# zsc/MOSS-TTSD

Measured on AMD Instinct MI355X. Metric: audio codec tokens/sec/node (decode, bf16, batch 32 @ 4k ctx), higher is better.
Workload: dtype bf16; 1 GPU; configs[2]: batch 32 synthetic dialogues/GPU, 4k-token KV context, top-k/top-p sampling on 8 channels, decode steps at full context; batch_per_gpu=32, context=4096, prompt=512, layers=28, hidden=2048, parallelism=dp1 (batch shard, no per-step collective)

## Files before the change

include/mtts.h:

```cpp
#ifndef MTTS_H
#define MTTS_H

#include <stdint.h>

#ifdef __cplusplus
extern "C" {
#endif

#define MTTS_OK 0
#define MTTS_EINVAL (-1)
#define MTTS_EHIP (-2)
#define MTTS_ENOMEM (-3)
#define MTTS_ESTATE (-4)

#define MTTS_CHANNELS 8

typedef struct MttsConfig {
    int32_t vocab_size;
    int32_t hidden_size;
    int32_t intermediate_size;
    int32_t num_hidden_layers;
    int32_t num_attention_heads;
    int32_t num_key_value_heads;
    int32_t head_dim;
// ... 66 lines not shown
                      const MttsSamplerCfg* sampler, uint64_t seed,
                      int64_t* host_out_ids, int32_t out_capacity, int32_t* out_len,
                      const int64_t* host_forced, int32_t forced_len, int64_t* host_decisions,
                      void* stream);

int32_t mtts_begin(MttsEngine* e, const int64_t* host_input_ids, const uint8_t* host_attention_mask,
                   int32_t B, int32_t T, int32_t max_length,
                   const MttsSamplerCfg* sampler, uint64_t seed, void* stream);
int32_t mtts_step(MttsEngine* e, int32_t n_steps, void* stream);
int32_t mtts_sync_state(MttsEngine* e, int32_t* steps_done, int32_t* all_finished, void* stream);
int32_t mtts_read_generated(MttsEngine* e, int64_t* host_gen, int32_t capacity_steps, int32_t* n_steps);
int32_t mtts_set_output_scores(MttsEngine* e, int32_t on);
int32_t mtts_read_scores(MttsEngine* e, float* host_lp, int32_t capacity_steps, int32_t* n_steps);
int32_t mtts_slot_read_scores(MttsEngine* e, int32_t slot, float* host_rows, int32_t capacity_steps, int32_t* n_steps);
int32_t mtts_set_top_logprobs(MttsEngine* e, int32_t k);
int32_t mtts_read_top_logprobs(MttsEngine* e, float* host_logp, int32_t* host_top_ids, float* host_top_logp,
                               int32_t capacity_steps, int32_t* n_steps);
int32_t mtts_slot_read_top_logprobs(MttsEngine* e, int32_t slot, float* host_logp, int32_t* host_top_ids, float* host_top_logp,
                                    int32_t capacity_steps, int32_t* n_steps);
int32_t mtts_score(MttsEngine* e, const int64_t* host_input_ids, const uint8_t* host_attention_mask,
                   const int64_t* host_labels, int32_t B, int32_t T, float* host_logp, void* stream);
#define MTTS_SCORE_MAX_TOPK 16
#define MTTS_SCORE_TOPK_ROWS 512
int32_t mtts_score_topk(MttsEngine* e, const int64_t* host_input_ids, const uint8_t* host_attention_mask,
                        const int64_t* host_labels, int32_t B, int32_t T, float* host_logp, int32_t k,
                        int32_t* host_top_ids, float* host_top_logp, void* stream);
int32_t mtts_read_logits(MttsEngine* e, uint16_t* host_logits0, uint16_t* host_logits17, void* stream);
int32_t mtts_read_logits_f32(MttsEngine* e, float* host_logits0, float* host_logits17, void* stream);
int32_t mtts_sched_open(MttsEngine* e, int32_t B, int32_t gen_cap, const MttsSamplerCfg* sampler, void* stream);
int32_t mtts_slot_submit(MttsEngine* e, int32_t slot, const int64_t* host_ids, int32_t T, int32_t max_length, uint64_t seed,
                         void* stream);
int32_t mtts_slot_submit_row(MttsEngine* e, int32_t slot, const int64_t* host_ids, int32_t T, int32_t max_length, uint64_t seed,
                             int32_t row_id, void* stream);
int32_t mtts_set_row_ids(MttsEngine* e, const int32_t* host_row_ids, int32_t n);
int32_t mtts_set_takes(MttsEngine* e, int32_t n);
int32_t mtts_set_sampler_floors(MttsEngine* e, const MttsSamplerFloors floors[8] );
int32_t mtts_set_sampler_bans(MttsEngine* e, const MttsSamplerBans bans[8] );
int32_t mtts_set_sampler_typical(MttsEngine* e, const float typical_p[8] );
int64_t mtts_debug_ban_launches(void);
int32_t mtts_slot_fork(MttsEngine* e, int32_t src_slot, int32_t dst_slot, uint64_t seed, int32_t row_id, void* stream);
int32_t mtts_slot_states(MttsEngine* e, int32_t* host_state, void* stream);
int32_t mtts_slot_read(MttsEngine* e, int32_t slot, int64_t* host_rows, int32_t capacity_steps, int32_t* n_steps);
int32_t mtts_read_seq_state(MttsEngine* e, int32_t* host_nas, int32_t* host_unfinished, int32_t* host_kv_len, void* stream);
int32_t mtts_slot_evict(MttsEngine* e, int32_t slot, void* stream);
int32_t mtts_kv_pool_state(MttsEngine* e, int32_t* total_pages, int32_t* free_pages, int32_t* max_pages_per_seq);
int32_t mtts_read_page_table(MttsEngine* e, int32_t* host_table, int32_t* host_n_pages);
int32_t mtts_set_forced_mode(MttsEngine* e, int32_t as_draw);
int32_t mtts_debug_read_device_page_table(MttsEngine* e, int32_t* host_table, void* stream);
int32_t mtts_export_codes(MttsEngine* e, int32_t first, int32_t n, int64_t* dev_codes, void* stream);
int32_t mtts_profile_enable(MttsEngine* e, int32_t on);
int32_t mtts_profile_read(MttsEngine* e, int32_t which, double* total_ms, int64_t* launches, int64_t* bytes);

int32_t mtts_debug_set_kv_len(MttsEngine* e, int32_t kv_len);
int32_t mtts_debug_kv_pack_stats(MttsEngine* e, int64_t* out6);
int32_t mtts_debug_step_plan(MttsEngine* e, int32_t pages_bound, char* buf, int32_t cap);
int32_t mtts_k_attn_bench(MttsEngine* e, int32_t phase, int32_t iters, float* avg_ms, int64_t* bytes_per_launch);
int32_t mtts_k_gemm_bench(int32_t N, int32_t K, int32_t epi, int32_t ksplit, int32_t waves, int32_t copies,
                          int32_t iters, float* avg_us);

int32_t mtts_debug_wseal_stats(MttsEngine* e, int64_t* out12);
int64_t mtts_debug_wseal_launches(void);
int32_t mtts_k_gemm_sealed_bench(const void* dev_w, int32_t N, int32_t K, int32_t epi, int32_t ksplit, int32_t copies,
                                 int32_t iters, int32_t sealed, int32_t head_form, float* avg_us, int64_t* out2);

int32_t mtts_k_wseal(const void* dev_packed, int32_t ntiles, int32_t K, int32_t ktw, void* dev_sealed, void* stream);
int32_t mtts_k_gemm_sealed(const void* dev_w, const void* dev_x, void* dev_out, int32_t M, int32_t N, int32_t K, int32_t epi,
                           int32_t ksplit, int32_t sealed, int32_t head_form, int64_t* out2, void* stream);
int32_t mtts_k_gemm_bf16(const void* dev_w, const void* dev_x, void* dev_y,
                         int32_t M, int32_t N, int32_t K, int32_t ksplit, void* stream);
int64_t mtts_debug_gemm_depth_launches(void);
int64_t mtts_debug_fold_norm_launches(void);
int32_t mtts_k_oproj_resid(const void* dev_wo, const void* dev_attn, void* dev_x, void* dev_x_packed, int32_t R, int32_t N,
                           void* stream);
int32_t mtts_k_fold_pair(const void* dev_wo, const void* dev_attn, void* dev_x, const void* dev_norm_w, const void* dev_wgu,
                         float eps, int32_t R, int32_t N_gu, void* dev_y, void* stream);
int32_t mtts_k_bf16_round_check(int64_t* out2, void* stream);
int32_t mtts_k_fold_bench(int32_t N_gu, int32_t copies, int32_t iters, int32_t mode, float* avg_us);
int64_t mtts_debug_attn_row_launches(void);
int32_t mtts_k_attn_section(const float* dev_slabs, int32_t ksplit, const void* dev_qnw, const void* dev_knw, const void* dev_cos,
                            const void* dev_sin, float eps, const void* dev_k, const void* dev_v, const int32_t* host_lens,
                            const int32_t* host_page_table, int32_t R, int32_t Lmax, int32_t nq, int32_t nkv, int32_t sealed,
                            int32_t path, void* dev_out, void* dev_kcache, void* dev_vcache, void* dev_kpack, void* dev_vpack,
                            void* stream);
int32_t mtts_k_attn_prefill(const float* dev_slabs, int32_t ksplit, const void* dev_qnw, const void* dev_knw, const void* dev_cos,
                            const void* dev_sin, float eps, const void* dev_k, const void* dev_v, const int32_t* host_lens,
                            const int32_t* host_cached, const int32_t* host_page_table, int32_t B, int32_t Lmax, int32_t nq,
                            int32_t nkv, void* dev_out, void* dev_q, void* dev_kcache, void* dev_vcache, void* stream);
int32_t mtts_k_gemm_swiglu_bf16(const void* dev_w, const void* dev_x, void* dev_y,
                                int32_t M, int32_t N, int32_t K, void* stream);
int32_t mtts_k_rmsnorm(const void* dev_x, const void* dev_w, void* dev_y,
                       int32_t rows, int32_t n, float eps, void* stream);
int32_t mtts_k_embed_norm(const int32_t* host_tokens, const int32_t* host_seq, const void* const* host_tables,
                          const int32_t* host_vocab, const void* dev_norm_w, int32_t R, int32_t H, float eps,
                          void* dev_x, void* dev_xn, void* stream);
int32_t mtts_k_resid_norm(const float* dev_slabs, int32_t ksplit, int32_t Npad, void* dev_x, const void* dev_norm_w,
                          const int32_t* host_seq, const int32_t* host_last, int32_t R, int32_t H, int32_t nseq, float eps,
                          void* dev_xn, void* dev_hlast, void* stream);
int32_t mtts_k_gemv_small(int32_t epi, int32_t pro, const void* dev_w, int32_t rows, int32_t N, int32_t K, int32_t want_ksplit,
                          const void* dev_x_in, const float* dev_slabs, int32_t slab_ksplit, const void* dev_norm_w, float eps,
                          void* dev_x_out, const float* dev_opart, const int32_t* host_seq, const int32_t* host_pos, int32_t nq,
                          int32_t nchunks_max, const void* dev_xrows, void* dev_y, int32_t* out_plan, void* stream);
int32_t mtts_k_gemm_tile(int32_t epi, const void* dev_w, const void* dev_x, void* dev_y, int32_t M, int32_t N, int32_t K,
                         int32_t ksplit, void* stream);
int32_t mtts_k_rope_kvwrite(const void* dev_qkv, const int32_t* host_pos, const void* dev_qnorm, const void* dev_knorm,
                            const void* dev_cos, const void* dev_sin, int32_t R, int32_t nq, int32_t nkv, float eps,
                            void* dev_q, void* dev_k, void* dev_v, void* stream);
int32_t mtts_k_paged_attn_decode(const void* dev_q, const void* dev_k, const void* dev_v, const int32_t* host_lens,
                                 const int32_t* host_page_table, int32_t R, int32_t Lmax, int32_t nq, int32_t nkv,
                                 void* dev_out, void* stream);
int32_t mtts_k_kv_seal(const void* dev_pages, int32_t npages, void* dev_sealed, int32_t as_k, void* stream);
int32_t mtts_k_head_ce(const void* dev_w, const void* dev_x, const int32_t* host_labels, int32_t M, int32_t N, int32_t K,
                       int32_t n_valid, int32_t segments, float* dev_logp, void* stream);
int32_t mtts_k_head_topk(const void* dev_w, const void* dev_x, int32_t M, int32_t N, int32_t K, int32_t n_valid,
                         int32_t segments, int32_t k, int32_t* dev_ids, float* dev_logp, void* stream);
int32_t mtts_k_lora_pack(const void* dev_base, int32_t rows, int32_t cols, const float* dev_lora_a, const float* dev_lora_b,
                         int32_t r, float scaling, int32_t rows_pad, int32_t row_mul, int32_t row_off, int32_t dtype,
                         void* dev_out, void* stream);
int32_t mtts_k_lora_delta(const void* dev_x, int32_t R, int32_t K, int32_t Npad, int32_t nseg, const int32_t* host_segs,
                          int32_t n_adapters, const void* const* host_a, const void* const* host_b, const int32_t* host_r,
                          const float* host_scaling, const int32_t* host_row_adapter, float* dev_slabs, int32_t ks, void* stream);
int32_t mtts_k_swiglu_slabs(const void* dev_w, const void* dev_x, const float* dev_delta, void* dev_y, float* dev_slab0_out,
                            int32_t M, int32_t N, int32_t K, void* stream);
int32_t mtts_k_sample(const void* dev_logits_bf16, int32_t rows, int32_t vocab,
                      const void* dev_history_bitmap, const MttsSamplerCfg* cfg,
                      int32_t mask_id, uint64_t seed, int32_t step, int32_t channel,
                      int32_t* dev_tokens, void* stream);
int32_t mtts_k_sample_scores(const void* dev_logits_bf16, int32_t rows, int32_t vocab,
                             const void* dev_history_bitmap, const MttsSamplerCfg* cfg,
                             int32_t mask_id, uint64_t seed, int32_t step, int32_t channel,
                             int32_t* dev_tokens, float* dev_logp, void* stream);
int32_t mtts_k_sample_floors(const void* dev_logits_bf16, int32_t rows, int32_t vocab,
                             const void* dev_history_bitmap, const MttsSamplerCfg* cfg,
                             int32_t mask_id, uint64_t seed, int32_t step, int32_t channel,
                             int32_t* dev_tokens, float* dev_logp, const MttsSamplerFloors* floors, void* stream);
int32_t mtts_k_sample_bans(const void* dev_logits_bf16, int32_t rows, int32_t vocab,
                           const void* dev_history_bitmap, const MttsSamplerCfg* cfg,
                           int32_t mask_id, uint64_t seed, int32_t step, int32_t channel,
                           int32_t* dev_tokens, float* dev_logp, const MttsSamplerFloors* floors, const void* dev_ban,
                           void* stream);
int32_t mtts_k_sample_typical(const void* dev_logits_bf16, int32_t rows, int32_t vocab,
                              const void* dev_history_bitmap, const MttsSamplerCfg* cfg,
                              int32_t mask_id, uint64_t seed, int32_t step, int32_t channel,
                              int32_t* dev_tokens, float* dev_logp, const MttsSamplerFloors* floors, const void* dev_ban,
                              float typical_p, void* stream);
int32_t mtts_k_ngram_ban(const int32_t* dev_hist, const int32_t* dev_lens, int32_t rows, int32_t cap, int32_t n,
                         const int32_t* host_static, int32_t n_static, int32_t vocab, int32_t eos_id, int32_t eos_on,
                         void* dev_ban, void* stream);
int32_t mtts_k_gen_topk(const void* dev_logits, int32_t is_f32, int32_t rows, int32_t vocab, int32_t mask_id,
                        const int32_t* dev_decisions, int32_t k, float* dev_logp, int32_t* dev_top_ids, float* dev_top_logp,
                        void* stream);

typedef struct MttsCodecConfig {
    int32_t nq, codebook_size, rvq_dim, quant_out_dim;
    int32_t adapter_layers, adapter_dim, adapter_heads, adapter_ffn, adapter_max_pos;
    int32_t up_stride;
    int32_t dec_layers, dec_dim, dec_heads, dec_ffn, dec_max_pos, mel_bins;
    int32_t voc_dim, voc_inter, voc_layers, n_fft, hop;
    int32_t mel_n_fft, mel_hop, mel_frames;
    int32_t enc_layers, enc_dim, enc_heads, enc_ffn, enc_max_pos;
    int32_t sem_adapter_layers, pre_rvq_layers, down_pool;
} MttsCodecConfig;

typedef struct MttsCodec MttsCodec;
const char* mtts_codec_last_error(void);
int32_t mtts_codec_create(const MttsCodecConfig* cfg, int32_t device, MttsCodec** out);
int32_t mtts_codec_destroy(MttsCodec* c);
// ... 42 lines not shown
```

moss-ttsd_amd/csrc/attn.hip:

```cpp
#include "launch.h"
#include <algorithm>
#include <atomic>
#include <cstdlib>
#ifndef MTTS_PK_WAVES
#define MTTS_PK_WAVES 0
#endif
#if MTTS_PK_WAVES
#define PK_OCC(PK) __attribute__((amdgpu_waves_per_eu((PK) ? MTTS_PK_WAVES : 1, (PK) ? MTTS_PK_WAVES : 8)))
#else
#define PK_OCC(PK)
#endif

#include "seal.h"

__device__ bool seal_lane_k(const u32x4_t* __restrict__ raw, u32x4_t* __restrict__ pk, uint8_t* __restrict__ lds, int lane) {
    u32x4_t v[16];
#pragma unroll
    for (int j = 0; j < 16; ++j) v[j] = raw[j * 64];
    __builtin_amdgcn_wave_barrier();
    uint32_t* row = (uint32_t*)(lds + lane * 128);
#pragma unroll
    for (int j = 0; j < 16; ++j)
#pragma unroll
        for (int c = 0; c < 4; c += 2) {
            const uint32_t a = u4c(v[j], c), b = u4c(v[j], c + 1);
            row[2 * j + (c >> 1)] = ((a >> 7) & 0xffu) | (((a >> 23) & 0xffu) << 8) | (((b >> 7) & 0xffu) << 16) | (((b >> 23) & 0xffu) << 24);
        }
    __builtin_amdgcn_wave_barrier();
    uint32_t a0 = 0u, a1 = 0u, n0 = 0u, n1 = 0u;
    for (int t = 0; t < 64; ++t) {
        const uint32_t e = *(const uint16_t*)(lds + t * 128 + 2 * lane);
        a0 += e & 0xffu; n0 += (e & 0xffu) ? 1u : 0u;
        a1 += e >> 8; n1 += (e >> 8) ? 1u : 0u;
    }
    const int s0 = n0 ? min(max((int)((a0 + n0 / 2) / n0) - 125, -127), 127) : 0;
    const int s1 = n1 ? min(max((int)((a1 + n1 / 2) / n1) - 125, -127), 127) : 0;
    int8_t* sv = (int8_t*)(lds + 8192);
    sv[2 * lane] = (int8_t)s0;
    sv[2 * lane + 1] = (int8_t)s1;
    __builtin_amdgcn_wave_barrier();
    bool unfit = false;
#pragma unroll
    for (int j = 0; j < 16; ++j) {
        uint32_t w[4] = {v[j].x, v[j].y, v[j].z, v[j].w};
#pragma unroll
        for (int c = 0; c < 4; ++c) {
            const uint32_t sh = *(const uint16_t*)(sv + 8 * j + 2 * c);
            uint32_t out = 0u;
#pragma unroll
            for (int h = 0; h < 2; ++h) {
                uint32_t b = (w[c] >> (16 * h)) & 0xffffu;
                const int sft = (int)(int8_t)((sh >> (8 * h)) & 0xffu);
                const int e = (int)((b >> 7) & 0xffu);
                if (e == 0) {
                    if ((b & 0x7fu) && sft) unfit = true;
                } else {
                    const int e2 = e - sft;
                    if (e == 255 ? sft != 0 : (e2 < 1 || e2 > 254)) unfit = true;
                    else b = (b - ((uint32_t)sft << 7)) & 0xffffu;
                }
                out |= b << (16 * h);
            }
            w[c] = out;
        }
        v[j] = u32x4_t{w[0], w[1], w[2], w[3]};
    }
    return seal_encode(v, pk, ((uint32_t)s0 & 0xffu) | (((uint32_t)s1 & 0xffu) << 8), unfit);
}
__device__ bool seal_lane_v(const u32x4_t* __restrict__ raw, u32x4_t* __restrict__ pk, uint8_t* __restrict__ lds, int lane) {
    u32x4_t v[16];
#pragma unroll
    for (int j = 0; j < 16; ++j) v[j] = raw[j * 64];
    const int sub = lane >> 5;
    __builtin_amdgcn_wave_barrier();
    uint32_t* row = (uint32_t*)(lds + lane * 128);
#pragma unroll
    for (int it = 0; it < 16; ++it)
#pragma unroll
        for (int h = 0; h < 2; ++h) {
            uint32_t sum = 0u, cnt = 0u;
#pragma unroll
            for (int c = 0; c < 4; ++c) {
                const uint32_t e = (u4c(v[it], c) >> (7 + 16 * h)) & 0xffu;
                sum += e;
                cnt += e ? 1u : 0u;
            }
            row[2 * it + h] = sum | (cnt << 16);
        }
    __builtin_amdgcn_wave_barrier();
    int mean;
    {
        const int t = lane, st = (t >> 1) & 1, j = 2 * (t >> 2) + (t & 1);
        uint32_t tot = 0u, cn = 0u;
        for (int d = 0; d < 32; ++d) {
            const uint32_t w = ((const uint32_t*)(lds + (st * 32 + d) * 128))[j];
            tot += w & 0xffffu;
// ... 66 lines not shown
                              : seal_lane_k(kcache + layer * raw_layer + pi * (MTTS_PAGE * MTTS_HD / 8) + lane,
                                            kpack + layer * pk_layer + pi * (MTTS_PKU * 64) + lane, klds, lane);
        seal_count(fit, cnt, layer, wave, lane);
    }
}
__global__ __launch_bounds__(128) void kv_seal_all_kernel(const u32x4_t* __restrict__ kcache, const u32x4_t* __restrict__ vcache,
                                                          u32x4_t* __restrict__ kpack, u32x4_t* __restrict__ vpack, int total_pages,
                                                          size_t raw_layer, size_t pk_layer, unsigned long long* __restrict__ cnt) {
    __shared__ __attribute__((aligned(16))) uint8_t klds[8192 + 128];
    __shared__ __attribute__((aligned(16))) uint8_t vlds[8192 + 320];
    const int kvh = blockIdx.y, layer = blockIdx.z, wave = threadIdx.x >> 6, lane = threadIdx.x & 63;
    const size_t pi = (size_t)kvh * total_pages + blockIdx.x;
    const bool fit = wave ? seal_lane_v(vcache + layer * raw_layer + pi * (MTTS_PAGE * MTTS_HD / 8) + lane,
                                        vpack + layer * pk_layer + pi * (MTTS_PKU * 64) + lane, vlds, lane)
                          : seal_lane_k(kcache + layer * raw_layer + pi * (MTTS_PAGE * MTTS_HD / 8) + lane,
                                        kpack + layer * pk_layer + pi * (MTTS_PKU * 64) + lane, klds, lane);
    seal_count(fit, cnt, layer, wave, lane);
}
__global__ __launch_bounds__(64) void kv_seal_pages_kernel(const u32x4_t* __restrict__ raw, u32x4_t* __restrict__ pk, int as_k) {
    __shared__ __attribute__((aligned(16))) uint8_t klds[8192 + 320];
    const u32x4_t* src = raw + (size_t)blockIdx.x * (MTTS_PAGE * MTTS_HD / 8) + threadIdx.x;
    u32x4_t* dst = pk + (size_t)blockIdx.x * (MTTS_PKU * 64) + threadIdx.x;
    if (as_k == 1) seal_lane_k(src, dst, klds, threadIdx.x);
    else if (as_k == 2) seal_lane_v(src, dst, klds, threadIdx.x);
    else seal_lane(src, dst);
}
void launch_kv_seal_pages(const void* raw, void* pk, int npages, int as_k, hipStream_t st) {
    hipLaunchKernelGGL(kv_seal_pages_kernel, dim3(npages), dim3(64), 0, st, (const u32x4_t*)raw, (u32x4_t*)pk, as_k);
}
__global__ __launch_bounds__(64) void kv_pack_count_kernel(const u32x4_t* __restrict__ kpack, const u32x4_t* __restrict__ vpack,
                                                           const int32_t* __restrict__ page_table, const int32_t* __restrict__ complete,
                                                           int max_pages, int total_pages, size_t pk_layer, unsigned long long* __restrict__ out) {
    const int b = blockIdx.x, kvh = blockIdx.y, layer = blockIdx.z, lane = threadIdx.x;
    unsigned long long n = 0, dk = 0, dv = 0;
    for (int pg = 0; pg < complete[b]; ++pg) {
        const size_t pi = (size_t)kvh * total_pages + page_table[(size_t)b * max_pages + pg];
        const u32x4_t fk = kpack[layer * pk_layer + pi * (MTTS_PKU * 64) + 12 * 64 + lane];
        const u32x4_t fv = vpack[layer * pk_layer + pi * (MTTS_PKU * 64) + 12 * 64 + lane];
        n += 1;
        dk += __any(fk.w != 0u) ? 1 : 0;
        dv += __any(fv.w != 0u) ? 1 : 0;
    }
    if (lane == 0 && n) {
        atomicAdd(out + 0, n); atomicAdd(out + 1, dk); atomicAdd(out + 2, n); atomicAdd(out + 3, dv);
    }
}
void launch_kv_pack_count(const void* kpack, const void* vpack, const int32_t* page_table, const int32_t* complete, int B, int max_pages,
                          int total_pages, int nkv, int L, unsigned long long* out, hipStream_t st) {
    const size_t pk_layer = (size_t)total_pages * nkv * (MTTS_PKU * 64);
    hipLaunchKernelGGL(kv_pack_count_kernel, dim3(B, nkv, L), dim3(64), 0, st, (const u32x4_t*)kpack, (const u32x4_t*)vpack, page_table,
                       complete, max_pages, total_pages, pk_layer, out);
}
void launch_kv_seal_rows(const void* kcache, const void* vcache, void* kpack, void* vpack, const int32_t* page_table,
                         const RowMeta* meta, int R, int max_pages, int total_pages, int nkv, int L, unsigned long long* cnt, hipStream_t st) {
    const size_t raw_layer = (size_t)total_pages * nkv * (MTTS_PAGE * MTTS_HD / 8), pk_layer = (size_t)total_pages * nkv * (MTTS_PKU * 64);
    hipLaunchKernelGGL(kv_seal_scan_kernel, dim3((R + 63) / 64, nkv, L), dim3(128), 0, st, (const u32x4_t*)kcache, (const u32x4_t*)vcache,
                       (u32x4_t*)kpack, (u32x4_t*)vpack, page_table, meta, R, max_pages, total_pages, raw_layer, pk_layer, cnt);
}
void launch_kv_seal_all(const void* kcache, const void* vcache, void* kpack, void* vpack, int total_pages, int nkv, int L,
                        unsigned long long* cnt, hipStream_t st) {
    const size_t raw_layer = (size_t)total_pages * nkv * (MTTS_PAGE * MTTS_HD / 8), pk_layer = (size_t)total_pages * nkv * (MTTS_PKU * 64);
    hipLaunchKernelGGL(kv_seal_all_kernel, dim3(total_pages, nkv, L), dim3(128), 0, st, (const u32x4_t*)kcache, (const u32x4_t*)vcache,
                       (u32x4_t*)kpack, (u32x4_t*)vpack, total_pages, raw_layer, pk_layer, cnt);
}


__device__ __forceinline__ void fuse_reduce(const QkvFuse& f, int r, int col, int lane, float& a, float& b) {
    const size_t kstride = (size_t)MTTS_PFCAP * f.Npad;
    const float* p0 = f.partial + (size_t)r * f.Npad + col + lane;
    a = 0.f; b = 0.f;
    for (int k0 = 0; k0 < f.ksplit; k0 += 8) {
        float ta[8], tb[8];
#pragma unroll
        for (int j = 0; j < 8; ++j) {
            const float* pk = p0 + (size_t)min(k0 + j, f.ksplit - 1) * kstride;
            ta[j] = pk[0];
            tb[j] = pk[64];
        }
        if (k0 == 0) { a = ta[0]; b = tb[0]; }
#pragma unroll
        for (int j = 0; j < 8; ++j)
            if (k0 + j < f.ksplit && k0 + j > 0) { a += ta[j]; b += tb[j]; }
    }
    a = rbf(a);
    b = rbf(b);
}

__device__ __forceinline__ void fuse_reduce_request(const QkvFuse& f, int r, int col, int lane, float (&ta)[8], float (&tb)[8]) {
    const size_t kstride = (size_t)MTTS_PFCAP * f.Npad;
    const float* p0 = f.partial + (size_t)r * f.Npad + col + lane;
#pragma unroll
    for (int j = 0; j < 8; ++j) {
        const float* pk = p0 + (size_t)min(j, f.ksplit - 1) * kstride;
        ta[j] = pk[0];
        tb[j] = pk[64];
    }
}
__device__ __forceinline__ void fuse_reduce_sum(const QkvFuse& f, const float (&ta)[8], const float (&tb)[8], float& a, float& b) {
    a = ta[0]; b = tb[0];
#pragma unroll
    for (int j = 1; j < 8; ++j)
        if (j < f.ksplit) { a += ta[j]; b += tb[j]; }
    a = rbf(a);
    b = rbf(b);
}

struct FuseVec { float w0, w1, c, s; };
__device__ __forceinline__ FuseVec fuse_load_vec(const QkvFuse& f, const uint16_t* __restrict__ nw, int pos, int lane) {
    FuseVec v;
    v.w0 = bf2f(nw[lane]);
    v.w1 = bf2f(nw[lane + 64]);
    v.c = bf2f(f.rope_cos[(size_t)pos * 64 + lane]);
    v.s = bf2f(f.rope_sin[(size_t)pos * 64 + lane]);
    return v;
}
__device__ __forceinline__ void fuse_norm_rope(const QkvFuse& f, const FuseVec& v, float a, float b, float& o1, float& o2) {
    const float ss = wave_sum(a * a + b * b);
    const float inv = 1.0f / sqrtf(ss / (float)MTTS_HD + f.eps);
    a = rbf(v.w0 * rbf(a * inv));
    b = rbf(v.w1 * rbf(b * inv));
    o1 = rbf(rbf(a * v.c) + rbf(-b * v.s));
    o2 = rbf(rbf(b * v.c) + rbf(a * v.s));
}

template <int G, bool FUSED, bool PK>
__global__ __launch_bounds__(256) PK_OCC(PK) void attn_scores_kernel(
    const uint16_t* __restrict__ qbuf, u32x4_t* __restrict__ kcache, const int32_t* __restrict__ page_table,
    const RowMeta* __restrict__ meta, uint16_t* __restrict__ scores, float* __restrict__ stats, int max_pages,
    int total_pages, int nq, int nkv, float scale, QkvFuse f, const u32x4_t* __restrict__ kpack) {
    __shared__ __attribute__((aligned(16))) uint32_t qs[G][MTTS_HD / 2];
    __shared__ __attribute__((aligned(16))) uint16_t knew[MTTS_HD];
    __shared__ __attribute__((aligned(16))) uint32_t qw[PK ? 4 : 1][G][MTTS_HD / 2];
    const int r = blockIdx.z, kvh = blockIdx.y;
    const RowMeta m = meta[r];
    if (m.seq < 0) return;
    const int len = m.pos + 1;
    const int npages = (len + MTTS_PAGE - 1) / MTTS_PAGE;
    if ((int)blockIdx.x * 4 >= npages) return;
    const int wave = __builtin_amdgcn_readfirstlane(threadIdx.x >> 6), lane = threadIdx.x & 63;
    const int pg = blockIdx.x * 4 + wave;
    const int own_pg = m.pos >> 6;
    const int Lmax = max_pages * MTTS_PAGE;
    uint32_t qreg[(G * MTTS_HD / 2 + 255) / 256];
    if (!FUSED) {
#pragma unroll
        for (int i = 0; i < (G * MTTS_HD / 2 + 255) / 256; ++i) {
            const int idx = threadIdx.x + 256 * i;
            qreg[i] = idx < G * MTTS_HD / 2 ? ((const uint32_t*)qbuf)[((size_t)r * nq + kvh * G) * (MTTS_HD / 2) + idx] : 0u;
        }
    }
    const bool own = FUSED && (own_pg >> 2) == (int)blockIdx.x;
    const bool pre = FUSED && f.ksplit <= 8 && wave < G + (own ? 1 : 0);
    float pta[8], ptb[8];
    FuseVec pfv{0.f, 0.f, 0.f, 0.f};
    if (pre) {
        const bool isk = wave == G;
        pfv = fuse_load_vec(f, isk ? f.knorm_w : f.qnorm_w, m.pos, lane);
        fuse_reduce_request(f, r, (isk ? nq + kvh : kvh * G + wave) * MTTS_HD, lane, pta, ptb);
    }
    const int page = pg < npages ? page_table[(size_t)m.seq * max_pages + pg] : 0;
    const u32x4_t* kp = kcache + ((size_t)kvh * total_pages + page) * (MTTS_PAGE * MTTS_HD / 8) + lane;

    auto stage_q = [&]() {
        if (FUSED) {
            for (int hh = wave; hh < G + (own ? 1 : 0); hh += 4) {
                const bool isk = hh == G;
                float a, b, o1, o2;
                FuseVec fv;
                if (pre && hh == wave) {
                    fv = pfv;
                    fuse_reduce_sum(f, pta, ptb, a, b);
                } else {
                    fv = fuse_load_vec(f, isk ? f.knorm_w : f.qnorm_w, m.pos, lane);
                    fuse_reduce(f, r, (isk ? nq + kvh : kvh * G + hh) * MTTS_HD, lane, a, b);
                }
                fuse_norm_rope(f, fv, a, b, o1, o2);
                if (!isk) {
                    ((uint16_t*)qs[hh])[lane] = f2bf(o1);
                    ((uint16_t*)qs[hh])[lane + 64] = f2bf(o2);
                } else {
                    knew[lane] = f2bf(o1);
                    knew[lane + 64] = f2bf(o2);
                    const int opage = page_table[(size_t)m.seq * max_pages + own_pg];
                    uint16_t* base = (uint16_t*)kcache + ((size_t)kvh * total_pages + opage) * (MTTS_PAGE * MTTS_HD);
                    const int tok = m.pos & 63;
                    base[(((lane >> 3) * 64) + tok) * 8 + (lane & 7)] = f2bf(o1);
                    base[((((lane + 64) >> 3) * 64) + tok) * 8 + (lane & 7)] = f2bf(o2);
                }
            }
        } else {
#pragma unroll
            for (int i = 0; i < (G * MTTS_HD / 2 + 255) / 256; ++i) {
                const int idx = threadIdx.x + 256 * i;
                if (idx < G * MTTS_HD / 2) (&qs[0][0])[idx] = qreg[i];
            }
        }
        __syncthreads();
    };
    auto finish = [&](const float* acc) {
        const int tok = pg * MTTS_PAGE + lane;
        const bool valid = tok < len;
#pragma unroll
        for (int g = 0; g < G; ++g) {
            const int h = kvh * G + g;
            float sc = rbf(rbf(acc[g]) * scale);
            if (valid) scores[((size_t)r * nq + h) * Lmax + tok] = f2bf(sc);
            float mx = wave_max(valid ? sc : -INFINITY);
            float e = valid ? expf(sc - mx) : 0.f;
            float sm = wave_sum(e);
            if (lane == 0) {
                float* st = stats + (((size_t)r * nq + h) * max_pages + pg) * 2;
                st[0] = mx;
                st[1] = sm;
            }
        }
    };
    auto raw_dots = [&](u32x4_t (&kv)[16]) {
        if (FUSED && pg == own_pg && lane == (m.pos & 63)) {
#pragma unroll
            for (int j = 0; j < 16; ++j) kv[j] = *(const u32x4_t*)&knew[8 * j];
        }
        float acc[G];
#pragma unroll
        for (int g = 0; g < G; ++g) acc[g] = 0.f;
#pragma unroll
        for (int j = 0; j < 16; ++j) {
#pragma unroll
            for (int g = 0; g < G; ++g) {
                const u32x4_t q = *(const u32x4_t*)&qs[g][4 * j];
                acc[g] = dot2bf(kv[j].x, q.x, acc[g]);
                acc[g] = dot2bf(kv[j].y, q.y, acc[g]);
                acc[g] = dot2bf(kv[j].z, q.z, acc[g]);
                acc[g] = dot2bf(kv[j].w, q.w, acc[g]);
            }
#pragma unroll
            for (int g = 0; g < G; ++g) asm volatile("" : "+v"(acc[g]));
            if ((j & 3) == 3) __builtin_amdgcn_sched_barrier(0);
        }
        finish(acc);
    };

    if (PK && pg < own_pg) {
        u32x4_t pk[MTTS_PKU];
        const u32x4_t* pp = kpack + ((size_t)kvh * total_pages + page) * (MTTS_PKU * 64) + lane;
#pragma unroll
        for (int j = 0; j < MTTS_PKU; ++j) pk[pk_order(j)] = __builtin_nontemporal_load(pp + pk_order(j) * 64);
        stage_q();
        bool qok = true;
        const uint32_t sh = pk[12].z;
#pragma unroll
        for (int g = 0; g < G; ++g) {
            const uint32_t qd = qs[g][lane];
            uint32_t out = 0u;
#pragma unroll
            for (int h = 0; h < 2; ++h) {
                uint32_t b = (qd >> (16 * h)) & 0xffffu;
                const int sft = (int)(int8_t)((sh >> (8 * h)) & 0xffu);
                if ((b & 0x7fffu) && sft) {
                    const int e = (int)((b >> 7) & 0xffu), e2 = e + sft;
                    if (e == 0 || e == 255 || e2 < 1 || e2 > 254) qok = false;
                    else b = (b + ((uint32_t)sft << 7)) & 0xffffu;
                }
                out |= b << (16 * h);
            }
            qw[PK ? wave : 0][g][lane] = out;
        }
        __builtin_amdgcn_wave_barrier();
        if (__any(pk[12].w != 0u || !qok)) {
            u32x4_t kv[16];
#pragma unroll
            for (int j = 0; j < 16; ++j) kv[j] = __builtin_nontemporal_load(kp + j * 64);
            raw_dots(kv);
            return;
        }
        float acc[G];
#pragma unroll
        for (int g = 0; g < G; ++g) acc[g] = 0.f;
#pragma unroll
        for (int j = 0; j < 16; ++j) {
            uint32_t w[4];
            pk_unit(pk, j, w);
#pragma unroll
            for (int g = 0; g < G; ++g) {
                const u32x4_t q = *(const u32x4_t*)&qw[PK ? wave : 0][g][4 * j];
                acc[g] = dot2bf(w[0], q.x, acc[g]);
                acc[g] = dot2bf(w[1], q.y, acc[g]);
                acc[g] = dot2bf(w[2], q.z, acc[g]);
                acc[g] = dot2bf(w[3], q.w, acc[g]);
            }
#pragma unroll
            for (int g = 0; g < G; ++g) asm volatile("" : "+v"(acc[g]));
            if ((j & 3) == 3) __builtin_amdgcn_sched_barrier(0);
        }
        finish(acc);
    } else {
        u32x4_t kv[16];
#pragma unroll
        for (int j = 0; j < 16; ++j) kv[j] = __builtin_nontemporal_load(kp + j * 64);
        stage_q();
        if (pg >= npages) return;
        raw_dots(kv);
    }
}

template <int G, bool FUSED, bool PK, bool SF>
__global__ __launch_bounds__(PV_WAVES * 64) PK_OCC(PK) void attn_pv_kernel(
    const uint16_t* __restrict__ scores, const float* __restrict__ stats, u32x4_t* __restrict__ vcache,
    const int32_t* __restrict__ page_table, const RowMeta* __restrict__ meta, float* __restrict__ opart,
    int max_pages, int total_pages, int nchunks_max, int nq, int nkv, QkvFuse f, const u32x4_t* __restrict__ vpack) {
    __shared__ float red[PV_WAVES][G][MTTS_HD];
    __shared__ uint16_t pbuf[PV_WAVES][G][MTTS_PAGE];
    __shared__ __attribute__((aligned(16))) uint16_t vnew[MTTS_HD];
    const int r = blockIdx.z, kvh = blockIdx.y, chunk = blockIdx.x;
    const RowMeta m = meta[r];
    if (m.seq < 0) return;
    const int len = m.pos + 1;
    const int npages = (len + MTTS_PAGE - 1) / MTTS_PAGE;
    if (chunk * ATT_PB >= npages) return;
    const int wave = threadIdx.x >> 6, lane = threadIdx.x & 63;
    const int Lmax = max_pages * MTTS_PAGE;
    const int sub = lane >> 5, dl = lane & 31;
    float2 s0[G];
    if (SF) {
#pragma unroll
        for (int g = 0; g < G; ++g) {
            const float* st = stats + ((size_t)r * nq + kvh * G + g) * max_pages * 2;
            s0[g] = lane < npages ? *(const float2*)(st + 2 * lane) : float2{-INFINITY, 0.f};
        }
        __builtin_amdgcn_sched_barrier(0);
    }
    u32x4_t vv[16];
    int pg = chunk * ATT_PB + wave * (ATT_PB / PV_WAVES);
    const int own_pg = m.pos >> 6;
    bool packed = false;
    const u32x4_t* vp = nullptr;
    uint16_t sraw[G];
    auto load_page = [&]() {
        if (SF) {
            const int tok = pg * MTTS_PAGE + lane;
#pragma unroll
            for (int g = 0; g < G; ++g) sraw[g] = tok < len ? scores[((size_t)r * nq + kvh * G + g) * Lmax + tok] : (uint16_t)0;
            __builtin_amdgcn_sched_barrier(0);
        }
        const int page = page_table[(size_t)m.seq * max_pages + pg];
        vp = vcache + ((size_t)kvh * total_pages + page) * (MTTS_PAGE * MTTS_HD / 8) + lane;
        packed = PK && pg < own_pg;
        if (packed) {
            const u32x4_t* pp = vpack + ((size_t)kvh * total_pages + page) * (MTTS_PKU * 64) + lane;
#pragma unroll
            for (int it = 0; it < MTTS_PKU; ++it) vv[pk_order(it)] = __builtin_nontemporal_load(pp + pk_order(it) * 64);
        } else {
#pragma unroll
            for (int it = 0; it < 16; ++it) vv[it] = __builtin_nontemporal_load(vp + it * 64);
        }
    };
    const bool own_wave = FUSED && own_pg >= pg && own_pg < pg + ATT_PB / PV_WAVES;
    const bool pre_v = SF && own_wave && f.ksplit <= 8;
    float vta[8], vtb[8];
    if (pre_v) fuse_reduce_request(f, r, (nq + nkv + kvh) * MTTS_HD, lane, vta, vtb);
    if (pg < npages) load_page();
    if (own_wave) {
        float a, b;
        if (pre_v) fuse_reduce_sum(f, vta, vtb, a, b);
        else fuse_reduce(f, r, (nq + nkv + kvh) * MTTS_HD, lane, a, b);
        vnew[lane] = f2bf(a);
        vnew[lane + 64] = f2bf(b);
        const int page = page_table[(size_t)m.seq * max_pages + own_pg];
        const int tok = m.pos & 63;
        uint16_t* dst = (uint16_t*)vcache + ((size_t)kvh * total_pages + page) * (MTTS_PAGE * MTTS_HD) + (size_t)(tok >> 1) * (MTTS_HD * 2) + (tok & 1);
        dst[2 * lane] = f2bf(a);
        dst[2 * (lane + 64)] = f2bf(b);
    }
    float M[G], S[G];
#pragma unroll
    for (int g = 0; g < G; ++g) {
        const float* st = stats + ((size_t)r * nq + kvh * G + g) * max_pages * 2;
        float mx = -INFINITY;
        if (SF) mx = fmaxf(mx, s0[g].x);
        for (int p = lane + (SF ? 64 : 0); p < npages; p += 64) mx = fmaxf(mx, st[2 * p]);
        mx = wave_max(mx);
        float sm = 0.f;
        if (SF && lane < npages) sm += s0[g].y * expf(s0[g].x - mx);
        for (int p = lane + (SF ? 64 : 0); p < npages; p += 64) sm += st[2 * p + 1] * expf(st[2 * p] - mx);
        sm = wave_sum(sm);
        M[g] = mx;
        S[g] = sm;
    }
    float acc[G][4];
#pragma unroll
    for (int g = 0; g < G; ++g)
#pragma unroll
        for (int i = 0; i < 4; ++i) acc[g][i] = 0.f;
#pragma unroll 1
    for (int pp = 0; pp < ATT_PB / PV_WAVES; ++pp, ++pg) {
        if (pg >= npages) break;
        if (pp > 0) load_page();
        if (own_wave && pg == own_pg) {
            __builtin_amdgcn_wave_barrier();
            const int tp = (m.pos & 63) >> 1;
            if (sub == (tp & 1)) {
                const uint32_t w01 = ((const uint32_t*)vnew)[2 * dl], w23 = ((const uint32_t*)vnew)[2 * dl + 1];
                const uint32_t nv[4] = {w01 & 0xffffu, w01 >> 16, w23 & 0xffffu, w23 >> 16};
                const bool hi = m.pos & 1;
#pragma unroll
                for (int it = 0; it < 16; ++it)
                    if (it == (tp >> 1)) {
                        vv[it].x = hi ? (vv[it].x & 0xffffu) | (nv[0] << 16) : (vv[it].x & 0xffff0000u) | nv[0];
                        vv[it].y = hi ? (vv[it].y & 0xffffu) | (nv[1] << 16) : (vv[it].y & 0xffff0000u) | nv[1];
                        vv[it].z = hi ? (vv[it].z & 0xffffu) | (nv[2] << 16) : (vv[it].z & 0xffff0000u) | nv[2];
                        vv[it].w = hi ? (vv[it].w & 0xffffu) | (nv[3] << 16) : (vv[it].w & 0xffff0000u) | nv[3];
                    }
            }
        }
        uint16_t pun[G];
        bool pok = true;
        {
            const int tok = pg * MTTS_PAGE + lane;
            const int sv = (PK && packed) ? (int)(vv[12].z & 0xffu) : 0;
#pragma unroll
            for (int g = 0; g < G; ++g) {
                float p = 0.f;
                if (tok < len) {
                    float s = bf2f(SF ? sraw[g] : scores[((size_t)r * nq + kvh * G + g) * Lmax + tok]);
                    p = expf(s - M[g]) / S[g];
                }
                uint32_t pb = f2bf(p);
                pun[g] = (uint16_t)pb;
                if (sv && (pb & 0x7fffu)) {
                    if (((pb >> 7) & 0xffu) == 0u) pok = false;
                    else pb += (uint32_t)sv << 7;
                }
                pbuf[wave][g][lane] = (uint16_t)pb;
            }
        }
        __builtin_amdgcn_wave_barrier();
        if (PK && packed && __any(vv[12].w != 0u || !pok)) {
            packed = false;
#pragma unroll
            for (int it = 0; it < 16; ++it) vv[it] = __builtin_nontemporal_load(vp + it * 64);
#pragma unroll
            for (int g = 0; g < G; ++g) pbuf[wave][g][lane] = pun[g];
            __builtin_amdgcn_wave_barrier();
        }
        if (PK && packed) {
#pragma unroll
            for (int it = 0; it < 16; ++it) {
                uint32_t w[4];
                pk_unit(vv, it, w);
#pragma unroll
                for (int g = 0; g < G; ++g) {
                    const uint32_t pp2 = ((const uint32_t*)&pbuf[wave][g][0])[it * 2 + sub];
                    acc[g][0] = dot2bf(w[0], pp2, acc[g][0]);
                    acc[g][1] = dot2bf(w[1], pp2, acc[g][1]);
                    acc[g][2] = dot2bf(w[2], pp2, acc[g][2]);
                    acc[g][3] = dot2bf(w[3], pp2, acc[g][3]);
                }
            }
        } else {
#pragma unroll
            for (int it = 0; it < 16; ++it) {
#pragma unroll
                for (int g = 0; g < G; ++g) {
                    const uint32_t pp2 = ((const uint32_t*)&pbuf[wave][g][0])[it * 2 + sub];
                    acc[g][0] = dot2bf(vv[it].x, pp2, acc[g][0]);
                    acc[g][1] = dot2bf(vv[it].y, pp2, acc[g][1]);
                    acc[g][2] = dot2bf(vv[it].z, pp2, acc[g][2]);
                    acc[g][3] = dot2bf(vv[it].w, pp2, acc[g][3]);
                }
            }
        }
        __builtin_amdgcn_wave_barrier();
    }
#pragma unroll
    for (int g = 0; g < G; ++g)
#pragma unroll
        for (int i = 0; i < 4; ++i) {
            float v = acc[g][i];
            v = add_xor32(v);
            if (sub == 0) red[wave][g][dl * 4 + i] = v;
        }
    __syncthreads();
    for (int i = threadIdx.x; i < G * MTTS_HD; i += PV_WAVES * 64) {
        int g = i / MTTS_HD, d = i % MTTS_HD;
        float v = red[0][g][d];
#pragma unroll
        for (int w = 1; w < PV_WAVES; ++w) v += red[w][g][d];
        opart[(((size_t)r * nq + kvh * G + g) * nchunks_max + chunk) * MTTS_HD + d] = v;
    }
}

__global__ __launch_bounds__(512) void attn_combine_kernel(const float* __restrict__ opart, const RowMeta* __restrict__ meta,
                                                           uint16_t* __restrict__ out_packed, int nchunks_max, int nq,
                                                           int pages_per_chunk) {
    const int r = blockIdx.x, h = blockIdx.y * 4 + (threadIdx.x >> 7), d = threadIdx.x & 127;
    if (h >= nq) return;
    const RowMeta m = meta[r];
    float s = 0.f;
    const int npages = m.seq >= 0 ? (m.pos + 1 + MTTS_PAGE - 1) / MTTS_PAGE : 0;
    const int nch = (npages + pages_per_chunk - 1) / pages_per_chunk;
    const float* p = opart + ((size_t)r * nq + h) * nchunks_max * MTTS_HD + d;
    for (int c0 = 0; c0 < nch; c0 += 8) {
        float t[8];
#pragma unroll
        for (int j = 0; j < 8; ++j) t[j] = p[(size_t)min(c0 + j, nch - 1) * MTTS_HD];
#pragma unroll
        for (int j = 0; j < 8; ++j)
            if (c0 + j < nch) s += t[j];
    }
    out_packed[xpack_off(r, h * MTTS_HD + d, nq * MTTS_HD)] = f2bf(s);
}

static_assert(ROW_WAVES >= 6 && ROW_WAVES <= 16, "one wave per q head + the K row + the V row; at most 1024 threads");
static std::atomic<long long> g_row_launches{0};
long long mtts_attn_row_launches() { return g_row_launches.load(); }

template <int G, bool PK>
__global__ __launch_bounds__(ROW_WAVES * 64) void attn_row_kernel(
    u32x4_t* __restrict__ kcache, u32x4_t* __restrict__ vcache, const int32_t* __restrict__ page_table,
    const RowMeta* __restrict__ meta, uint16_t* __restrict__ out_packed, int npb, int max_pages, int total_pages, int nq,
    int nkv, float scale, QkvFuse f, const u32x4_t* __restrict__ kpack, const u32x4_t* __restrict__ vpack) {
    constexpr int W = ROW_WAVES;
    extern __shared__ __attribute__((aligned(16))) uint8_t row_lds[];
    uint32_t* qs = (uint32_t*)row_lds;
    uint16_t* knew = (uint16_t*)(row_lds + G * 256);
    uint16_t* vnew = knew + MTTS_HD;
    uint32_t* qw = (uint32_t*)(row_lds + G * 256 + 512);
    uint16_t* pbuf = (uint16_t*)((uint8_t*)qw + (PK ? W * G * 256 : 0));
    float2* st = (float2*)((uint8_t*)pbuf + W * G * 128);
    uint16_t* sc = (uint16_t*)(st + G * npb);
    float* items = (float*)(sc + (size_t)G * npb * MTTS_PAGE);
    const int r = blockIdx.y, kvh = blockIdx.x;
    const RowMeta m = meta[r];
    if (m.seq < 0) {
        for (int i = threadIdx.x; i < G * MTTS_HD; i += W * 64) out_packed[xpack_off(r, kvh * G * MTTS_HD + i, nq * MTTS_HD)] = f2bf(0.f);
        return;
    }
    const int len = m.pos + 1;
    const int npages = min((len + MTTS_PAGE - 1) / MTTS_PAGE, npb);
    const int nch = (npages + ATT_PB - 1) / ATT_PB;
    const int wave = __builtin_amdgcn_readfirstlane(threadIdx.x >> 6), lane = threadIdx.x & 63;
    const int own_pg = m.pos >> 6;
    const int sub = lane >> 5, dl = lane & 31;
    const int32_t* ptab = page_table + (size_t)m.seq * max_pages;

    const bool epi = wave < G + 2;
    const int vw = epi ? wave + W - (G + 2) : wave - (G + 2);
    if (epi) {
        const int col = (wave < G ? kvh * G + wave : wave == G ? nq + kvh : nq + nkv + kvh) * MTTS_HD;
        FuseVec pfv{0.f, 0.f, 0.f, 0.f};
        if (wave <= G) pfv = fuse_load_vec(f, wave == G ? f.knorm_w : f.qnorm_w, m.pos, lane);
        float a, b;
        if (f.ksplit <= 8) {
            float pta[8], ptb[8];
            fuse_reduce_request(f, r, col, lane, pta, ptb);
            fuse_reduce_sum(f, pta, ptb, a, b);
        } else fuse_reduce(f, r, col, lane, a, b);
        const int opage = ptab[own_pg], tok = m.pos & 63;
        if (wave <= G) {
            float o1, o2;
            fuse_norm_rope(f, pfv, a, b, o1, o2);
            if (wave < G) {
                ((uint16_t*)(qs + wave * 64))[lane] = f2bf(o1);
                ((uint16_t*)(qs + wave * 64))[lane + 64] = f2bf(o2);
            } else {
                knew[lane] = f2bf(o1);
                knew[lane + 64] = f2bf(o2);
                uint16_t* base = (uint16_t*)kcache + ((size_t)kvh * total_pages + opage) * (MTTS_PAGE * MTTS_HD);
                base[(((lane >> 3) * 64) + tok) * 8 + (lane & 7)] = f2bf(o1);
                base[((((lane + 64) >> 3) * 64) + tok) * 8 + (lane & 7)] = f2bf(o2);
            }
        } else {
            vnew[lane] = f2bf(a);
            vnew[lane + 64] = f2bf(b);
            uint16_t* dst = (uint16_t*)vcache + ((size_t)kvh * total_pages + opage) * (MTTS_PAGE * MTTS_HD) + (size_t)(tok >> 1) * (MTTS_HD * 2) + (tok & 1);
            dst[2 * lane] = f2bf(a);
            dst[2 * (lane + 64)] = f2bf(b);
        }
        __builtin_amdgcn_sched_barrier(0);
    }
    auto stage = [&]() { __syncthreads(); };

    auto finish = [&](int pg, const float* acc) {
        const int tok = pg * MTTS_PAGE + lane;
        const bool valid = tok < len;
#pragma unroll
        for (int g = 0; g < G; ++g) {
            float s = rbf(rbf(acc[g]) * scale);
            if (valid) sc[(size_t)g * npb * MTTS_PAGE + tok] = f2bf(s);
            float mx = wave_max(valid ? s : -INFINITY);
            float e = valid ? expf(s - mx) : 0.f;
            float sm = wave_sum(e);
            if (lane == 0) st[g * npb + pg] = float2{mx, sm};
        }
    };
    auto raw_dots = [&](int pg, u32x4_t (&kv)[16]) {
        if (pg == own_pg && lane == (m.pos & 63)) {
#pragma unroll
            for (int j = 0; j < 16; ++j) kv[j] = *(const u32x4_t*)&knew[8 * j];
        }
        float acc[G];
#pragma unroll
        for (int g = 0; g < G; ++g) acc[g] = 0.f;
#pragma unroll
        for (int j = 0; j < 16; ++j) {
#pragma unroll
            for (int g = 0; g < G; ++g) {
                const u32x4_t q = *(const u32x4_t*)&qs[g * 64 + 4 * j];
                acc[g] = dot2bf(kv[j].x, q.x, acc[g]);
                acc[g] = dot2bf(kv[j].y, q.y, acc[g]);
                acc[g] = dot2bf(kv[j].z, q.z, acc[g]);
                acc[g] = dot2bf(kv[j].w, q.w, acc[g]);
            }
#pragma unroll
            for (int g = 0; g < G; ++g) asm volatile("" : "+v"(acc[g]));
            if ((j & 3) == 3) __builtin_amdgcn_sched_barrier(0);
        }
        finish(pg, acc);
    };
    auto k_page = [&](int pg, bool first) {
        const int page = ptab[pg];
        const u32x4_t* kp = kcache + ((size_t)kvh * total_pages + page) * (MTTS_PAGE * MTTS_HD / 8) + lane;
        if (PK && pg < own_pg) {
            u32x4_t pk[MTTS_PKU];
            const u32x4_t* pp = kpack + ((size_t)kvh * total_pages + page) * (MTTS_PKU * 64) + lane;
#pragma unroll
            for (int j = 0; j < MTTS_PKU; ++j) pk[pk_order(j)] = __builtin_nontemporal_load(pp + pk_order(j) * 64);
            if (first) stage();
            bool qok = true;
            const uint32_t sh = pk[12].z;
            uint32_t* qwv = qw + wave * G * 64;
            __builtin_amdgcn_wave_barrier();
#pragma unroll
            for (int g = 0; g < G; ++g) {
                const uint32_t qd = qs[g * 64 + lane];
                uint32_t out = 0u;
#pragma unroll
                for (int h = 0; h < 2; ++h) {
                    uint32_t b = (qd >> (16 * h)) & 0xffffu;
                    const int sft = (int)(int8_t)((sh >> (8 * h)) & 0xffu);
                    if ((b & 0x7fffu) && sft) {
                        const int e = (int)((b >> 7) & 0xffu), e2 = e + sft;
                        if (e == 0 || e == 255 || e2 < 1 || e2 > 254) qok = false;
                        else b = (b + ((uint32_t)sft << 7)) & 0xffffu;
                    }
                    out |= b << (16 * h);
                }
                qwv[g * 64 + lane] = out;
            }
            __builtin_amdgcn_wave_barrier();
            if (__any(pk[12].w != 0u || !qok)) {
                u32x4_t kv[16];
#pragma unroll
                for (int j = 0; j < 16; ++j) kv[j] = __builtin_nontemporal_load(kp + j * 64);
                raw_dots(pg, kv);
                return;
            }
            float acc[G];
#pragma unroll
            for (int g = 0; g < G; ++g) acc[g] = 0.f;
#pragma unroll
            for (int j = 0; j < 16; ++j) {
                uint32_t w[4];
                pk_unit(pk, j, w);
#pragma unroll
                for (int g = 0; g < G; ++g) {
                    const u32x4_t q = *(const u32x4_t*)&qwv[g * 64 + 4 * j];
                    acc[g] = dot2bf(w[0], q.x, acc[g]);
                    acc[g] = dot2bf(w[1], q.y, acc[g]);
                    acc[g] = dot2bf(w[2], q.z, acc[g]);
                    acc[g] = dot2bf(w[3], q.w, acc[g]);
                }
#pragma unroll
                for (int g = 0; g < G; ++g) asm volatile("" : "+v"(acc[g]));
                if ((j & 3) == 3) __builtin_amdgcn_sched_barrier(0);
            }
            finish(pg, acc);
        } else {
            u32x4_t kv[16];
#pragma unroll
            for (int j = 0; j < 16; ++j) kv[j] = __builtin_nontemporal_load(kp + j * 64);
            if (first) stage();
            raw_dots(pg, kv);
        }
    };
    if (vw < npages) k_page(vw, true);
    else stage();
#pragma unroll 1
    for (int pg = vw + W; pg < npages; pg += W) k_page(pg, false);

    u32x4_t vv[16];
    bool packed = false;
    const u32x4_t* vp = nullptr;
    auto load_page = [&](int pg) {
        const int page = ptab[pg];
        vp = vcache + ((size_t)kvh * total_pages + page) * (MTTS_PAGE * MTTS_HD / 8) + lane;
        packed = PK && pg < own_pg;
        if (packed) {
            const u32x4_t* pp = vpack + ((size_t)kvh * total_pages + page) * (MTTS_PKU * 64) + lane;
#pragma unroll
            for (int it = 0; it < MTTS_PKU; ++it) vv[pk_order(it)] = __builtin_nontemporal_load(pp + pk_order(it) * 64);
        } else {
#pragma unroll
            for (int it = 0; it < 16; ++it) vv[it] = __builtin_nontemporal_load(vp + it * 64);
        }
    };
    if (2 * wave < npages) load_page(2 * wave);
    __syncthreads();
    float M[G], S[G];
#pragma unroll
    for (int g = 0; g < G; ++g) {
        const float2* sg = st + g * npb;
        const float2 s0 = lane < npages ? sg[lane] : float2{-INFINITY, 0.f};
        float mx = -INFINITY;
        mx = fmaxf(mx, s0.x);
        for (int p = lane + 64; p < npages; p += 64) mx = fmaxf(mx, sg[p].x);
        mx = wave_max(mx);
        float sm = 0.f;
        if (lane < npages) sm += s0.y * expf(s0.x - mx);
        for (int p = lane + 64; p < npages; p += 64) sm += sg[p].y * expf(sg[p].x - mx);
        sm = wave_sum(sm);
        M[g] = mx;
        S[g] = sm;
    }
    uint16_t* pb = pbuf + wave * G * MTTS_PAGE;
#pragma unroll 1
    for (int item = wave; item < PV_WAVES * nch; item += W) {
        float acc[G][4];
#pragma unroll
        for (int g = 0; g < G; ++g)
#pragma unroll
            for (int i = 0; i < 4; ++i) acc[g][i] = 0.f;
#pragma unroll 1
        for (int pp = 0; pp < ATT_PB / PV_WAVES; ++pp) {
            const int pg = item * (ATT_PB / PV_WAVES) + pp;
            if (pg >= npages) break;
            if (pp > 0 || item != wave) load_page(pg);
            if (pg == own_pg) {
                const int tp = (m.pos & 63) >> 1;
                if (sub == (tp & 1)) {
                    const uint32_t w01 = ((const uint32_t*)vnew)[2 * dl], w23 = ((const uint32_t*)vnew)[2 * dl + 1];
                    const uint32_t nv[4] = {w01 & 0xffffu, w01 >> 16, w23 & 0xffffu, w23 >> 16};
                    const bool hi = m.pos & 1;
#pragma unroll
                    for (int it = 0; it < 16; ++it)
                        if (it == (tp >> 1)) {
                            vv[it].x = hi ? (vv[it].x & 0xffffu) | (nv[0] << 16) : (vv[it].x & 0xffff0000u) | nv[0];
                            vv[it].y = hi ? (vv[it].y & 0xffffu) | (nv[1] << 16) : (vv[it].y & 0xffff0000u) | nv[1];
                            vv[it].z = hi ? (vv[it].z & 0xffffu) | (nv[2] << 16) : (vv[it].z & 0xffff0000u) | nv[2];
                            vv[it].w = hi ? (vv[it].w & 0xffffu) | (nv[3] << 16) : (vv[it].w & 0xffff0000u) | nv[3];
                        }
                }
            }
            uint16_t pun[G];
            bool pok = true;
            {
                const int tok = pg * MTTS_PAGE + lane;
                const int sv = (PK && packed) ? (int)(vv[12].z & 0xffu) : 0;
#pragma unroll
                for (int g = 0; g < G; ++g) {
                    float p = 0.f;
                    if (tok < len) {
                        float s = bf2f(sc[(size_t)g * npb * MTTS_PAGE + tok]);
                        p = expf(s - M[g]) / S[g];
                    }
                    uint32_t pbits = f2bf(p);
                    pun[g] = (uint16_t)pbits;
                    if (sv && (pbits & 0x7fffu)) {
                        if (((pbits >> 7) & 0xffu) == 0u) pok = false;
                        else pbits += (uint32_t)sv << 7;
                    }
                    pb[g * MTTS_PAGE + lane] = (uint16_t)pbits;
                }
            }
            __builtin_amdgcn_wave_barrier();
            if (PK && packed && __any(vv[12].w != 0u || !pok)) {
                packed = false;
#pragma unroll
// ... 170 lines not shown
            sm = add_xor32(sm);
            M[g] = mx;
            S[g] = sm;
        }
        f32x16_t acc[GP][4];
#pragma unroll
        for (int g = 0; g < GP; ++g)
#pragma unroll
            for (int db = 0; db < 4; ++db)
#pragma unroll
                for (int i = 0; i < 16; ++i) acc[g][db][i] = 0.f;
#pragma unroll 1
        for (int pg = chunk * ATT_PF; pg < pg_end; ++pg) {
            const int page = page_table[(size_t)m0.seq * max_pages + pg];
            const uint32_t* vp = vcache + ((size_t)kvh * total_pages + page) * (MTTS_PAGE * MTTS_HD / 2) + (lane & 31);
            u32x4_t sv[4][GP];
#pragma unroll
            for (int ts = 0; ts < 4; ++ts) {
                const int tok0 = pg * MTTS_PAGE + ts * 16 + 8 * half;
#pragma unroll
                for (int g = 0; g < GP; ++g) {
                    sv[ts][g] = u32x4_t{0u, 0u, 0u, 0u};
                    if (tok0 <= pos) sv[ts][g] = *(const u32x4_t*)(scores + ((size_t)row * nq + kvh * G + g0 + g) * Lmax + tok0);
                }
            }
#pragma unroll
            for (int ts = 0; ts < 4; ++ts) {
                const int t0 = ts * 16 + 8 * half;
                u32x4_t va[4];
#pragma unroll
                for (int db = 0; db < 4; ++db) {
                    const uint32_t* q = vp + db * 32 + (size_t)(t0 / 2) * MTTS_HD;
                    va[db].x = q[0];
                    va[db].y = q[MTTS_HD];
                    va[db].z = q[2 * MTTS_HD];
                    va[db].w = q[3 * MTTS_HD];
                }
                const int tok0 = pg * MTTS_PAGE + t0;
#pragma unroll
                for (int g = 0; g < GP; ++g) {
                    const uint32_t sw[4] = {sv[ts][g].x, sv[ts][g].y, sv[ts][g].z, sv[ts][g].w};
                    uint32_t pw[4];
#pragma unroll
                    for (int j = 0; j < 4; ++j) {
                        const float p0 = (tok0 + 2 * j <= pos) ? expf(bflo(sw[j]) - M[g]) / S[g] : 0.f;
                        const float p1 = (tok0 + 2 * j + 1 <= pos) ? expf(bfhi(sw[j]) - M[g]) / S[g] : 0.f;
                        pw[j] = pack2(p0, p1);
                    }
                    u32x4_t pb = {pw[0], pw[1], pw[2], pw[3]};
#pragma unroll
                    for (int db = 0; db < 4; ++db)
                        acc[g][db] = __builtin_amdgcn_mfma_f32_32x32x16_bf16(*(bf16x8_t*)&va[db], *(bf16x8_t*)&pb, acc[g][db], 0, 0, 0);
                }
            }
        }
        if (mr.seq >= 0) {
#pragma unroll
            for (int g = 0; g < GP; ++g) {
                float* o = opart + (((size_t)row * nq + kvh * G + g0 + g) * nchunks_pf + chunk) * MTTS_HD + 4 * half;
#pragma unroll
                for (int db = 0; db < 4; ++db)
#pragma unroll
                    for (int q = 0; q < 4; ++q) {
                        const float4 v4 = make_float4(acc[g][db][4 * q], acc[g][db][4 * q + 1], acc[g][db][4 * q + 2], acc[g][db][4 * q + 3]);
                        *(float4*)(o + db * 32 + 8 * q) = v4;
                    }
            }
        }
    }
}

static bool pv_stats_first() {
    static int v = -1;
    if (v < 0) {
        const char* g = getenv("MTTS_PV_STATS_FIRST");
        v = (g && atoi(g) == 0) ? 0 : 1;
    }
    return v != 0;
}
template <int G>
static void launch_attn_g(const void* qbuf, void* kcache, void* vcache, const int32_t* page_table,
                          const RowMeta* meta, void* scores, float* stats, float* opart, void* out_packed, int R,
                          int pages_bound, int max_pages, int total_pages, int nchunks_max, int nq, int nkv, float scale,
                          const QkvFuse* fuse, AttnPhase phase, hipStream_t st, const KvPack* pack) {
    if (phase == ATTN_PF_SCORES) {
        dim3 ga((pages_bound + 3) / 4, nkv, R / MTTS_MAXR);
        hipLaunchKernelGGL((attn_prefill_scores_kernel<G>), ga, dim3(256), 0, st, (const uint16_t*)qbuf, (const u32x4_t*)kcache,
                           page_table, meta, (uint16_t*)scores, stats, max_pages, total_pages, nq, nkv, scale);
        return;
    }
    const int nchunks_pf = (max_pages + ATT_PF - 1) / ATT_PF;
    if (phase == ATTN_PF_PV) {
        dim3 gb((pages_bound + 4 * ATT_PF - 1) / (4 * ATT_PF), nkv, R / MTTS_MAXR);
        hipLaunchKernelGGL((attn_prefill_pv_kernel<G>), gb, dim3(256), 0, st, (const uint16_t*)scores, (const float*)stats,
                           (const uint32_t*)vcache, page_table, meta, opart, max_pages, total_pages, nchunks_pf, nq, nkv);
        return;
    }
    if (phase == ATTN_PF_COMBINE) {
        hipLaunchKernelGGL(attn_combine_kernel, dim3(R, (nq + 3) / 4), dim3(512), 0, st, (const float*)opart, meta,
                           (uint16_t*)out_packed, nchunks_pf, nq, ATT_PF);
        return;
    }
    const QkvFuse f = fuse ? *fuse : QkvFuse{nullptr, 0, 0, nullptr, nullptr, nullptr, nullptr, 0.f};
    const u32x4_t* kpk = pack ? (const u32x4_t*)pack->k : nullptr;
    const u32x4_t* vpk = pack ? (const u32x4_t*)pack->v : nullptr;
    if (phase == ATTN_ROW) {
        const size_t lds = (size_t)attn_row_lds_bytes(G, kpk != nullptr, pages_bound);
        if (kpk)
            hipLaunchKernelGGL((attn_row_kernel<G, true>), dim3(nkv, R), dim3(ROW_WAVES * 64), lds, st, (u32x4_t*)kcache, (u32x4_t*)vcache,
                               page_table, meta, (uint16_t*)out_packed, pages_bound, max_pages, total_pages, nq, nkv, scale, f, kpk, vpk);
        else
            hipLaunchKernelGGL((attn_row_kernel<G, false>), dim3(nkv, R), dim3(ROW_WAVES * 64), lds, st, (u32x4_t*)kcache, (u32x4_t*)vcache,
                               page_table, meta, (uint16_t*)out_packed, pages_bound, max_pages, total_pages, nq, nkv, scale, f, kpk, vpk);
        g_row_launches.fetch_add(1);
        return;
    }
#define MTTS_SC(FU, PK)                                                                                                  \
    hipLaunchKernelGGL((attn_scores_kernel<G, FU, PK>), ga, dim3(256), 0, st, (const uint16_t*)qbuf, (u32x4_t*)kcache, \
                       page_table, meta, (uint16_t*)scores, stats, max_pages, total_pages, nq, nkv, scale, f, kpk)
#define MTTS_PV2(FU, PK, SF)                                                                                                        \
    hipLaunchKernelGGL((attn_pv_kernel<G, FU, PK, SF>), gb, dim3(PV_WAVES * 64), 0, st, (const uint16_t*)scores, (const float*)stats, \
                       (u32x4_t*)vcache, page_table, meta, opart, max_pages, total_pages, nchunks_max, nq, nkv, f, vpk)
#define MTTS_PV(FU, PK)                        \
    do {                                       \
        if (pv_stats_first()) MTTS_PV2(FU, PK, true); \
        else MTTS_PV2(FU, PK, false);          \
    } while (0)
    if (phase == ATTN_ALL || phase == ATTN_SCORES) {
        dim3 ga((pages_bound + 3) / 4, nkv, R);
        if (fuse) { if (kpk) MTTS_SC(true, true); else MTTS_SC(true, false); }
        else { if (kpk) MTTS_SC(false, true); else MTTS_SC(false, false); }
    }
    if (phase == ATTN_ALL || phase == ATTN_PV) {
        dim3 gb((pages_bound + ATT_PB - 1) / ATT_PB, nkv, R);
        if (fuse) { if (vpk) MTTS_PV(true, true); else MTTS_PV(true, false); }
        else { if (vpk) MTTS_PV(false, true); else MTTS_PV(false, false); }
    }
#undef MTTS_SC
#undef MTTS_PV
#undef MTTS_PV2
    if (phase == ATTN_ALL || phase == ATTN_COMBINE)
        hipLaunchKernelGGL(attn_combine_kernel, dim3(R, (nq + 3) / 4), dim3(512), 0, st, (const float*)opart, meta,
                           (uint16_t*)out_packed, nchunks_max, nq, ATT_PB);
}

static int g_row_lds_max = 0;
bool attn_row_fits(int G, const QkvFuse* fuse, const KvPack* pack, int pages_bound) {
    const bool pk = pack && pack->k;
    if (!fuse || (G != 1 && G != 2 && G != 4) || pk != (pack && pack->v)) return false;
    return attn_row_lds_bytes(G, pk, pages_bound) <= g_row_lds_max;
}
int attn_row_prepare() {
    int dev = 0, cand[3] = {0, 0, 0};
    if (hipGetDevice(&dev) != hipSuccess) return -1;
    const hipDeviceAttribute_t attrs[3] = {hipDeviceAttributeMaxSharedMemoryPerMultiprocessor, hipDeviceAttributeSharedMemPerBlockOptin,
                                           hipDeviceAttributeMaxSharedMemoryPerBlock};
    for (int i = 0; i < 3; ++i)
        if (hipDeviceGetAttribute(&cand[i], attrs[i], dev) != hipSuccess) { cand[i] = 0; (void)hipGetLastError(); }
    std::sort(cand, cand + 3, [](int x, int y) { return x > y; });
    for (int i = 0; i < 3; ++i) {
        const int lim = cand[i];
        if (lim <= 0 || (i && lim == cand[i - 1])) continue;
        hipError_t e = hipSuccess;
#define MTTS_ROWP(GG, PK) \
    if (e == hipSuccess) e = hipFuncSetAttribute((const void*)attn_row_kernel<GG, PK>, hipFuncAttributeMaxDynamicSharedMemorySize, lim)
        MTTS_ROWP(1, false); MTTS_ROWP(1, true); MTTS_ROWP(2, false); MTTS_ROWP(2, true); MTTS_ROWP(4, false); MTTS_ROWP(4, true);
#undef MTTS_ROWP
        if (e == hipSuccess) { g_row_lds_max = lim; return 0; }
        (void)hipGetLastError();
    }
    return -1;
}
int attn_row_lds_limit() { return g_row_lds_max; }

int launch_attn(const void* qbuf, void* kcache, void* vcache, const int32_t* page_table,
                const RowMeta* meta, void* scores, float* stats, float* opart, void* out_packed, int R,
                int pages_bound, int max_pages, int total_pages, int nchunks_max, int nq, int nkv, float scale,
                const QkvFuse* fuse, AttnPhase phase, hipStream_t st, const KvPack* pack) {
    int G = nq / nkv;
    if (G != 1 && G != 2 && G != 4) return -1;
    if (phase == ATTN_ROW && !attn_row_fits(G, fuse, pack, pages_bound)) return -2;
#define MTTS_ATT(GG)                                                                                              \
    launch_attn_g<GG>(qbuf, kcache, vcache, page_table, meta, scores, stats, opart, out_packed, R, pages_bound,   \
                      max_pages, total_pages, nchunks_max, nq, nkv, scale, fuse, phase, st, pack)
    if (G == 1) MTTS_ATT(1);
    else if (G == 2) MTTS_ATT(2);
    else if (G == 4) MTTS_ATT(4);
    else return -1;
#undef MTTS_ATT
    return 0;
}
```

moss-ttsd_amd/csrc/engine.hip:

```cpp
#include "engine.h"
#include "staging.h"

#define FLUSH_STEPS 7
#define LINGER_STEPS 14
static inline int linger_bound(int B) { return 6 * B + 8; }

thread_local char g_err[512] = "";
int fail(int code, const char* fmt, ...) {
    va_list ap;
    va_start(ap, fmt);
    vsnprintf(g_err, sizeof(g_err), fmt, ap);
    va_end(ap);
    return code;
}

const char* mtts_last_error(void) { return g_err; }
int32_t mtts_version(void) { return 202; }

static auto ship_on(MttsEngine* e, hipStream_t st) {
    return [e, st](const PageEdits& ed) -> int {
        launch_set_pages(e->d_page_table, ed, st);
        HIPCHK(hipGetLastError());
        return 0;
    };
// ... 505 lines not shown
    e->mem.release(s);
    TRY(e->mem.get(&c, (size_t)rows * 64, false));
    TRY(e->mem.get(&s, (size_t)rows * 64, false));
    HIPCHK(hipMemcpyAsync(c, cosb, (size_t)rows * 64 * sizeof(T), hipMemcpyDeviceToDevice, st));
    HIPCHK(hipMemcpyAsync(s, sinb, (size_t)rows * 64 * sizeof(T), hipMemcpyDeviceToDevice, st));
    e->bufs.rope_rows = rows;
    return MTTS_OK;
}
int32_t mtts_bind_rope(MttsEngine* e, const void* cosb, const void* sinb, int32_t rows, void* stream) {
    if (!e || !cosb || !sinb || rows < 1) return fail(MTTS_EINVAL, "bad rope table");
    HIPCHK(hipSetDevice(e->device));
    if (e->f32) return bind_rope_tables(e, e->bufs.rope_cos_f, e->bufs.rope_sin_f, cosb, sinb, rows, S(stream));
    return bind_rope_tables(e, e->bufs.rope_cos, e->bufs.rope_sin, cosb, sinb, rows, S(stream));
}

static int wseal_policy(MttsEngine* e) {
    if (!e->wseal_dirty || !e->d_wseal_cnt) return MTTS_OK;
    HIPCHK(hipSetDevice(e->device));
    HIPCHK(hipDeviceSynchronize());
    HIPCHK(hipMemsetAsync(e->d_wseal_cnt, 0, WSEAL_KINDS * 2 * sizeof(unsigned long long), nullptr));
    const int H = e->H, I = e->I, Hp = round_up(H, 32);
    for (auto& l : e->layers) {
        if (l.wgu_s) launch_wseal_count(l.wgu_s, 2 * I, H, e->wseal_ktw[WSEAL_GU], e->d_wseal_cnt + 2 * WSEAL_GU, nullptr);
        if (l.wd_s) launch_wseal_count(l.wd_s, Hp, I, e->wseal_ktw[WSEAL_DOWN], e->d_wseal_cnt + 2 * WSEAL_DOWN, nullptr);
    }
    if (e->head0_s) launch_wseal_count(e->head0_s, e->V0_pad, H, e->wseal_ktw[WSEAL_HEAD0], e->d_wseal_cnt + 2 * WSEAL_HEAD0, nullptr);
    if (e->heads17_s) launch_wseal_count(e->heads17_s, 7 * e->Vs_pad, H, e->wseal_ktw[WSEAL_HEADS], e->d_wseal_cnt + 2 * WSEAL_HEADS, nullptr);
    HIPCHK(hipGetLastError());
    HIPCHK(hipMemcpyAsync(e->h_wseal_cnt, e->d_wseal_cnt, WSEAL_KINDS * 2 * sizeof(unsigned long long), hipMemcpyDeviceToHost, nullptr));
    HIPCHK(hipStreamSynchronize(nullptr));
    for (int k = 0; k < WSEAL_KINDS; ++k) {
        const unsigned long long groups = e->h_wseal_cnt[2 * k], bad = e->h_wseal_cnt[2 * k + 1];
        e->wseal_on[k] = e->wseal_ktw[k] && groups && (e->knobs.w_seal == 2 || (double)bad <= WSEAL_MAX_UNSEALED[k] * (double)groups);
    }
    e->wseal_dirty = false;
    return MTTS_OK;
}

int32_t mtts_weights_ready(MttsEngine* e) {
    if (!e) return fail(MTTS_EINVAL, "null engine");
    if (e->emb_bound != 0xff) return fail(MTTS_ESTATE, "embedding tables missing (mask %x)", e->emb_bound);
    if (!e->norm_bound) return fail(MTTS_ESTATE, "final norm missing");
    if (!e->bufs.rope_rows) return fail(MTTS_ESTATE, "rope table missing");
    for (int n = 0; n < e->L; ++n)
        if (e->layers[n].bound != 2047) return fail(MTTS_ESTATE, "layer %d incomplete (mask %x)", n, e->layers[n].bound);
    return wseal_policy(e);
}

static void prof_begin(MttsEngine* e, int which, hipStream_t st, hipEvent_t* a) {
    if (!e->prof) return;
    hipEvent_t s0, s1;
    hipEventCreate(&s0); hipEventCreate(&s1);
    hipEventRecord(s0, st);
    e->ev[which].push_back({s0, s1});
    *a = s1;
}
static void prof_end(MttsEngine* e, hipStream_t st, hipEvent_t a) {
    if (!e->prof) return;
    hipEventRecord(a, st);
}

static int pack_policy_reset(MttsEngine* e, hipStream_t st) {
    if (!e->d_seal_cnt) return 0;
    HIPCHK(hipMemsetAsync(e->d_seal_cnt, 0, (size_t)e->L * 4 * sizeof(unsigned long long), st));
    e->pack_k_on.assign(e->L, 1);
    e->pack_v_on.assign(e->L, 1);
    return 0;
}
static int attend_layer(MttsEngine* e, const StepPlan& plan, int n, const RowMeta* d_meta, int R, int pages_bound, int ks_qkv,
                        hipStream_t st, int64_t kv_tokens_hint) {
    static const AttnPhase decode_ph[3] = {ATTN_SCORES, ATTN_PV, ATTN_COMBINE}, prefill_ph[3] = {ATTN_PF_SCORES, ATTN_PF_PV, ATTN_PF_COMBINE};
    Layer& l = e->layers[n];
    const AttnForm form = plan.layers[n].attn;
    const float eps = e->cfg.rms_norm_eps, scale = 1.0f / sqrtf((float)MTTS_HD);
    uint16_t* kc = (uint16_t*)e->kcache + e->layer_stride * n;
    uint16_t* vc = (uint16_t*)e->vcache + e->layer_stride * n;
    const QkvFuse fz{e->bufs.partial, ks_qkv, e->qkv_rows, (const uint16_t*)l.qn, (const uint16_t*)l.kn, e->bufs.rope_cos, e->bufs.rope_sin, eps};
    const KvPack pk = layer_pack(e, plan, n);
    const KvPack* pkp = (pk.k || pk.v) ? &pk : nullptr;
    if (form == ATTN_FORM_ROW) {
        hipEvent_t ev = nullptr;
        prof_begin(e, PROF_SCORES, st, &ev);
        if (const int rc = launch_attn(e->qbuf, kc, vc, e->d_page_table, d_meta, e->scores, e->stats, e->opart, e->attn_p, R, pages_bound,
                                       e->max_pages, e->total_pages, e->nchunks_max, e->nq, e->nkv, scale, &fz, ATTN_ROW, st, pkp))
            return fail(MTTS_EINVAL, rc == -2 ? "the whole-row attention kernel does not take this launch" : "attention group size not built");
        prof_end(e, st, ev);
        if (e->prof) e->prof_bytes[PROF_SCORES] += 2 * kv_tokens_hint * e->nkv * MTTS_HD * 2;
        return 0;
    }
    const bool fused = form == ATTN_FORM_TWO_PASS_FUSED;
    const AttnPhase* ph = form == ATTN_FORM_PREFILL_MFMA ? prefill_ph : decode_ph;
    const int nphases = plan.path == PATH_SMALL ? 2 : 3;
    if (!fused)
        launch_qkv_post(e->bufs.partial, ks_qkv, e->qkv_rows, d_meta, l.qn, l.kn, e->bufs.rope_cos, e->bufs.rope_sin, e->qbuf,
                        kc, vc, e->d_page_table, e->max_pages, e->total_pages, R, e->nq, e->nkv, eps, st);
    for (int i = 0; i < nphases; ++i) {
        hipEvent_t ev = nullptr;
        if (i < 2) prof_begin(e, i == 0 ? PROF_SCORES : PROF_PV, st, &ev);
        if (launch_attn(e->qbuf, kc, vc, e->d_page_table, d_meta, e->scores, e->stats, e->opart, e->attn_p, R,
                        pages_bound, e->max_pages, e->total_pages, e->nchunks_max, e->nq, e->nkv, scale,
                        fused ? &fz : nullptr, ph[i], st, pkp))
            return fail(MTTS_EINVAL, "attention group size not built");
        if (i < 2) prof_end(e, st, ev);
    }
    if (e->prof) {
        e->prof_bytes[PROF_SCORES] += kv_tokens_hint * e->nkv * MTTS_HD * 2;
        e->prof_bytes[PROF_PV] += kv_tokens_hint * e->nkv * MTTS_HD * 2;
    }
    return 0;
}
static void seal_completed_pages(MttsEngine* e, const RowMeta* d_meta, int R, hipStream_t st) {
    if (e->kpack)
        launch_kv_seal_rows(e->kcache, e->vcache, e->kpack, e->vpack, e->d_page_table, d_meta, R, e->max_pages, e->total_pages, e->nkv, e->L, e->d_seal_cnt, st);
}

static int forward_small(MttsEngine* e, const StepPlan& plan, const RowMeta* d_meta, int pages_bound, hipStream_t st, int64_t kv_tokens_hint) {
    const int H = e->H, I = e->I, nq = e->nq, Hp = round_up(H, 32), R = MTTS_MAXR;
    const float eps = e->cfg.rms_norm_eps;
    uint16_t* xa = (uint16_t*)e->x;
    uint16_t* xb = (uint16_t*)e->x2;
    SmallPro base{};
    base.rows = plan.B; base.eps = eps; base.slab_npad = Hp;
    for (int n = 0; n < e->L; ++n) {
        Layer& l = e->layers[n];
        SmallPro pq = base;
        pq.x_in = xa; pq.x_out = xb; pq.slabs = e->partial2; pq.ksplit = n ? e->p_d.ksplit : 0; pq.norm_w = (const uint16_t*)l.ln_in;
        launch_gemv_small(EPI_PARTIAL, PRO_NORM, e->p_qkv, l.wqkv, H, e->qkv_rows, e->qkv_rows, e->bufs.partial, nullptr, pq, st);
        TRY(attend_layer(e, plan, n, d_meta, R, pages_bound, e->p_qkv.ksplit, st, kv_tokens_hint));
        SmallPro po = base;
        po.opart = e->opart; po.meta = d_meta; po.nchunks_max = e->nchunks_max; po.nq = nq; po.pages_per_chunk = ATT_PB;
        launch_gemv_small(EPI_PARTIAL, PRO_COMBINE, e->p_o, l.wo, nq * MTTS_HD, Hp, Hp, e->partial2, nullptr, po, st);
        SmallPro pg = base;
        pg.x_in = xb; pg.x_out = xa; pg.slabs = e->partial2; pg.ksplit = e->p_o.ksplit; pg.norm_w = (const uint16_t*)l.ln_post;
        launch_gemv_small(EPI_SILU_RM, PRO_NORM, e->p_gu, l.wgu, H, 2 * I, 2 * I, nullptr, (uint16_t*)e->act_rm, pg, st);
        SmallPro pd = base;
        pd.xrows = (const uint16_t*)e->act_rm;
        launch_gemv_small(EPI_PARTIAL, PRO_ROWS, e->p_d, l.wd, I, Hp, Hp, e->partial2, nullptr, pd, st);
    }
    seal_completed_pages(e, d_meta, R, st);
    SmallPro ph = base;
    ph.x_in = xa; ph.x_out = nullptr; ph.slabs = e->partial2; ph.ksplit = e->p_d.ksplit; ph.norm_w = (const uint16_t*)e->final_norm;
    launch_gemv_small(EPI_BF16, PRO_NORM, e->p_h0, e->head0, H, e->V0_pad, e->V0, nullptr, (uint16_t*)e->logits0, ph, st);
    launch_gemv_small(EPI_BF16, PRO_NORM, e->p_h17, e->heads17, H, 7 * e->Vs_pad, 7 * e->Vs_pad, nullptr, (uint16_t*)e->logits17, ph, st);
    HIPCHK(hipGetLastError());
    return MTTS_OK;
}

static int run_gemm(int epi, bool tiled, int R, int ks, bool sealed, int head_form, const GemmPlan& p, const void* Ws, const void* Wp,
                    const void* Xp, int K, int Npad, int n_valid, float* partial, uint16_t* out, hipStream_t st) {
    const int mb = (R + 31) / 32;
    if (tiled) launch_gemm_tile(epi, R, ks, Wp, Xp, K, Npad, n_valid, partial, out, st);
    else if (!sealed) launch_gemm(epi, mb, p, Wp, Xp, K, Npad, n_valid, partial, out, st);
    else if (!launch_gemm_sealed(epi, mb, p, Ws, Wp, Xp, K, Npad, n_valid, partial, out, head_form, st))
        return fail(MTTS_ESTATE, "the plan asks for a sealed weight read that the launcher does not take (K %d, N %d, %d row tiles)", K, Npad, mb);
    return 0;
}

static int forward_rows(MttsEngine* e, const StepPlan& plan, const int32_t* d_tokens, const RowMeta* d_meta, int pages_bound,
                        hipStream_t st, int64_t kv_tokens_hint) {
    const int H = e->H, I = e->I, nq = e->nq, nkv = e->nkv, R = plan.R, mb = plan.mb;
    const float eps = e->cfg.rms_norm_eps;
    const int Hp = round_up(H, 32);
    const bool tiled = plan.tiled, lora = plan.lora;
    if (plan.path == PATH_F32) return forward_rows_f32(e, d_tokens, d_meta, plan.heads == 1 ? plan.B : R, plan.heads, st);
    launch_embed_norm(d_tokens, d_meta, e->d_tables, e->layers[0].ln_in, e->x, e->xn, R, H, eps, st);
    if (plan.path == PATH_SMALL) return forward_small(e, plan, d_meta, pages_bound, st, kv_tokens_hint);
    if (lora && !e->bufs.d_bank) return fail(MTTS_ESTATE, "a pass with adapters on an engine without a bank");
// ... 1084 lines not shown
```

moss-ttsd_amd/csrc/hooks.hip:

```cpp
#include "engine.h"
#include "staging.h"

int32_t mtts_k_gemm_bf16(const void* w, const void* x, void* y, int32_t M, int32_t N, int32_t K, int32_t ksplit, void* stream) {
    if (!w || !x || !y || M < 1 || M > MTTS_PFCAP || K % 16 || N < 1) return fail(MTTS_EINVAL, "gemm: need 1<=M<=MTTS_PFCAP, K%%16==0");
    hipStream_t st = S(stream);
    int Npad = round_up(N, 32);
    void *wp = nullptr, *xp = nullptr;
    float* part = nullptr;
    GemmPlan p = mtts_plan_gemm(Npad, K, ksplit);
    p.depth = gemm_depth_env();
    DevBufs hb;
    TRY(hb.get((uint16_t**)&wp, (size_t)Npad * K));
    const bool tiled = M > MTTS_RCAP;
    const int ks = tiled ? (ksplit > 0 ? ksplit : mtts_tile_ksplit(Npad, K, M)) : p.ksplit;
    TRY(hb.get((uint16_t**)&xp, (size_t)MTTS_PFCAP * K));
    TRY(hb.get(&part, (size_t)ks * MTTS_PFCAP * Npad));
    launch_pack_weight(w, wp, N, K, Npad, 1, 0, st);
    const int tiles = (M + 31) / 32;
    launch_pack_rows(x, xp, M, K, tiles == 3 ? 4 : tiles, st);
    if (tiled) launch_gemm_tile(EPI_PARTIAL, M, ks, wp, xp, K, Npad, Npad, part, nullptr, st);
    else launch_gemm(EPI_PARTIAL, tiles, p, wp, xp, K, Npad, Npad, part, nullptr, st);
    launch_reduce_partial_bf16(part, y, ks, Npad, N, M, st);
    HIPCHK(hipGetLastError());
    HIPCHK(hipStreamSynchronize(st));
// ... 498 lines not shown
    DevBufs hb;
    TRY(hb.get(&slab, (size_t)MTTS_PFCAP * N));
    TRY(hb.get(&meta, R)); TRY(hb.get(&pt, (size_t)R * max_pages));
    TRY(hb.get(&kc, (size_t)total_pages * nkv * MTTS_PAGE * MTTS_HD)); TRY(hb.get(&vc, (size_t)total_pages * nkv * MTTS_PAGE * MTTS_HD));
    std::vector<RowMeta> hm(R);
    std::vector<int32_t> hpt((size_t)R * max_pages);
    for (int r = 0; r < R; ++r) { hm[r] = RowMeta{r, host_pos[r], 1, 0}; for (int p = 0; p < max_pages; ++p) hpt[(size_t)r * max_pages + p] = r * max_pages + p; }
    HIPCHK(hipMemcpy(meta, hm.data(), R * sizeof(RowMeta), hipMemcpyHostToDevice));
    HIPCHK(hipMemcpy(pt, hpt.data(), hpt.size() * 4, hipMemcpyHostToDevice));
    launch_bf16_to_f32(dev_qkv, slab, (size_t)R * N, st);
    launch_qkv_post(slab, 1, N, meta, dev_qnorm, dev_knorm, dev_cos, dev_sin, dev_q, kc, vc, pt, max_pages, total_pages, R, nq, nkv, eps, st);
    HIPCHK(hipGetLastError());
    HIPCHK(hipStreamSynchronize(st));
    std::vector<uint16_t> hk((size_t)total_pages * nkv * MTTS_PAGE * MTTS_HD), hv(hk.size()), ok((size_t)R * nkv * MTTS_HD), ov(ok.size());
    HIPCHK(hipMemcpy(hk.data(), kc, hk.size() * 2, hipMemcpyDeviceToHost));
    HIPCHK(hipMemcpy(hv.data(), vc, hv.size() * 2, hipMemcpyDeviceToHost));
    for (int r = 0; r < R; ++r)
        for (int h = 0; h < nkv; ++h)
            for (int d = 0; d < MTTS_HD; ++d) {
                const int page = r * max_pages + host_pos[r] / MTTS_PAGE, t = host_pos[r] % MTTS_PAGE;
                const size_t base = ((size_t)h * total_pages + page) * (MTTS_PAGE * MTTS_HD);
                ok[((size_t)r * nkv + h) * MTTS_HD + d] = hk[base + (((d >> 3) * 64) + t) * 8 + (d & 7)];
                ov[((size_t)r * nkv + h) * MTTS_HD + d] = hv[base + ((size_t)(t >> 1) * MTTS_HD + d) * 2 + (t & 1)];
            }
    HIPCHK(hipMemcpy(dev_k, ok.data(), ok.size() * 2, hipMemcpyHostToDevice));
    HIPCHK(hipMemcpy(dev_v, ov.data(), ov.size() * 2, hipMemcpyHostToDevice));
    return MTTS_OK;
}

int32_t mtts_k_paged_attn_decode(const void* dev_q, const void* dev_k, const void* dev_v, const int32_t* host_lens,
                                 const int32_t* host_page_table, int32_t R, int32_t Lmax, int32_t nq, int32_t nkv,
                                 void* dev_out, void* stream) {
    if (!dev_q || !dev_k || !dev_v || !host_lens || !dev_out || R < 1 || R > MTTS_MAXR || Lmax < 1 || nq < 1 || nkv < 1 || nq % nkv)
        return fail(MTTS_EINVAL, "paged_attn_decode: bad argument (1..32 rows)");
    hipStream_t st = S(stream);
    const int max_pages = pages_for(Lmax), total_pages = R * max_pages, nch = (max_pages + ATT_PB - 1) / ATT_PB;
    std::vector<int32_t> hpt((size_t)R * max_pages);
    std::vector<char> seen(total_pages, 0);
    for (size_t i = 0; i < hpt.size(); ++i) {
        hpt[i] = host_page_table ? host_page_table[i] : (int32_t)i;
        if (hpt[i] < 0 || hpt[i] >= total_pages || seen[hpt[i]]) return fail(MTTS_EINVAL, "page table must be a permutation of 0..%d", total_pages - 1);
        seen[hpt[i]] = 1;
    }
    std::vector<RowMeta> hm(MTTS_MAXR, RowMeta{-1, 0, 0, 0});
    int pages_bound = 1;
    for (int r = 0; r < R; ++r) {
        if (host_lens[r] < 1 || host_lens[r] > Lmax) return fail(MTTS_EINVAL, "row %d: length %d outside 1..%d", r, host_lens[r], Lmax);
        hm[r] = RowMeta{r, host_lens[r] - 1, 1, 0};
        pages_bound = std::max(pages_bound, pages_for(host_lens[r]));
    }
    RowMeta* meta = nullptr; int32_t *pt = nullptr, *lens = nullptr; uint16_t *kc = nullptr, *vc = nullptr, *scores = nullptr, *outp = nullptr;
    float *stats = nullptr, *opart = nullptr;
    const size_t cache_n = (size_t)total_pages * nkv * MTTS_PAGE * MTTS_HD;
    DevBufs hb;
    TRY(hb.get(&meta, MTTS_MAXR)); TRY(hb.get(&pt, hpt.size())); TRY(hb.get(&lens, R));
    TRY(hb.get(&kc, cache_n)); TRY(hb.get(&vc, cache_n));
    TRY(hb.get(&scores, (size_t)MTTS_MAXR * nq * max_pages * MTTS_PAGE));
    TRY(hb.get(&stats, (size_t)MTTS_MAXR * nq * max_pages * 2));
    TRY(hb.get(&opart, (size_t)MTTS_MAXR * nq * nch * MTTS_HD));
    TRY(hb.get(&outp, (size_t)MTTS_MAXR * nq * MTTS_HD));
    HIPCHK(hipMemcpy(meta, hm.data(), hm.size() * sizeof(RowMeta), hipMemcpyHostToDevice));
    HIPCHK(hipMemcpy(pt, hpt.data(), hpt.size() * 4, hipMemcpyHostToDevice));
    HIPCHK(hipMemcpy(lens, host_lens, R * 4, hipMemcpyHostToDevice));
    launch_pack_kv_pages(dev_k, dev_v, kc, vc, pt, lens, R, Lmax, nkv, max_pages, total_pages, st);
    KvPack pk{nullptr, nullptr};
    const char* g = getenv("MTTS_KV_PACK");
    if (!g || atoi(g) != 0) {
        uint8_t *kp = nullptr, *vp = nullptr;
        const size_t pk_n = (size_t)total_pages * nkv * MTTS_PKU * 64 * 16;
        TRY(hb.get(&kp, pk_n)); TRY(hb.get(&vp, pk_n));
        launch_kv_seal_all(kc, vc, kp, vp, total_pages, nkv, 1, nullptr, st);
        pk = KvPack{kp, vp};
    }
    const float scale = 1.0f / sqrtf((float)MTTS_HD);
    if (launch_attn(dev_q, kc, vc, pt, meta, scores, stats, opart, outp, MTTS_MAXR, pages_bound, max_pages, total_pages, nch, nq, nkv,
                    scale, nullptr, ATTN_ALL, st, pk.k ? &pk : nullptr))
        return fail(MTTS_EINVAL, "attention group size not built (1, 2, 4)");
    launch_unpack_rows(outp, dev_out, R, nq * MTTS_HD, st);
    HIPCHK(hipGetLastError());
    HIPCHK(hipStreamSynchronize(st));
    return MTTS_OK;
}

int32_t mtts_k_attn_section(const float* dev_slabs, int32_t ksplit, const void* dev_qnw, const void* dev_knw, const void* dev_cos,
                            const void* dev_sin, float eps, const void* dev_k, const void* dev_v, const int32_t* host_lens,
                            const int32_t* host_page_table, int32_t R, int32_t Lmax, int32_t nq, int32_t nkv, int32_t sealed,
                            int32_t path, void* dev_out, void* dev_kcache, void* dev_vcache, void* dev_kpack, void* dev_vpack,
                            void* stream) {
    if (!dev_slabs || !dev_qnw || !dev_knw || !dev_cos || !dev_sin || !dev_k || !dev_v || !host_lens || !dev_out || !dev_kcache ||
        !dev_vcache || R < 1 || R > MTTS_MAXR || Lmax < 1 || nq < 1 || nkv < 1 || nq % nkv || ksplit < 1 || (path != 0 && path != 1))
        return fail(MTTS_EINVAL, "attn_section: bad argument (1..32 rows, path 0 or 1)");
    hipStream_t st = S(stream);
    const int max_pages = pages_for(Lmax), total_pages = R * max_pages, nch = (max_pages + ATT_PB - 1) / ATT_PB;
    const int Npad = (nq + 2 * nkv) * MTTS_HD;
    std::vector<int32_t> hpt((size_t)R * max_pages);
    std::vector<char> seen(total_pages, 0);
    for (size_t i = 0; i < hpt.size(); ++i) {
        hpt[i] = host_page_table ? host_page_table[i] : (int32_t)i;
        if (hpt[i] < 0 || hpt[i] >= total_pages || seen[hpt[i]]) return fail(MTTS_EINVAL, "page table must be a permutation of 0..%d", total_pages - 1);
        seen[hpt[i]] = 1;
    }
    std::vector<RowMeta> hm(MTTS_MAXR, RowMeta{-1, 0, 0, 0});
    std::vector<int32_t> cached(R, 0);
    int pages_bound = 1;
    for (int r = 0; r < R; ++r) {
        if (host_lens[r] < 0 || host_lens[r] > Lmax) return fail(MTTS_EINVAL, "row %d: length %d outside 0..%d", r, host_lens[r], Lmax);
        if (!host_lens[r]) continue;
        hm[r] = RowMeta{r, host_lens[r] - 1, 1, 0};
        cached[r] = host_lens[r] - 1;
        pages_bound = std::max(pages_bound, pages_for(host_lens[r]));
    }
    pages_bound = std::min(round_up(pages_bound, ATT_PB), max_pages);
    RowMeta* meta = nullptr; int32_t *pt = nullptr, *lens = nullptr; uint16_t *kc = nullptr, *vc = nullptr, *scores = nullptr, *outp = nullptr;
    float *stats = nullptr, *opart = nullptr, *slabs = nullptr;
    uint8_t *kp = nullptr, *vp = nullptr;
    const size_t cache_n = (size_t)total_pages * nkv * MTTS_PAGE * MTTS_HD, pk_n = (size_t)total_pages * nkv * MTTS_PKU * 64 * 16;
    DevBufs hb;
    TRY(hb.get(&meta, MTTS_MAXR)); TRY(hb.get(&pt, hpt.size())); TRY(hb.get(&lens, R));
    TRY(hb.get(&kc, cache_n)); TRY(hb.get(&vc, cache_n));
    TRY(hb.get(&scores, (size_t)MTTS_MAXR * nq * max_pages * MTTS_PAGE));
    TRY(hb.get(&stats, (size_t)MTTS_MAXR * nq * max_pages * 2));
    TRY(hb.get(&opart, (size_t)MTTS_MAXR * nq * nch * MTTS_HD));
    TRY(hb.get(&outp, (size_t)MTTS_MAXR * nq * MTTS_HD));
    TRY(hb.get(&slabs, (size_t)ksplit * MTTS_PFCAP * Npad, false));
    HIPCHK(hipMemcpyAsync(meta, hm.data(), hm.size() * sizeof(RowMeta), hipMemcpyHostToDevice, st));
    HIPCHK(hipMemcpyAsync(pt, hpt.data(), hpt.size() * 4, hipMemcpyHostToDevice, st));
    HIPCHK(hipMemcpyAsync(lens, cached.data(), R * 4, hipMemcpyHostToDevice, st));
    for (int k = 0; k < ksplit; ++k)
        HIPCHK(hipMemcpyAsync(slabs + (size_t)k * MTTS_PFCAP * Npad, dev_slabs + (size_t)k * R * Npad, (size_t)R * Npad * 4, hipMemcpyDeviceToDevice, st));
    launch_pack_kv_pages(dev_k, dev_v, kc, vc, pt, lens, R, Lmax, nkv, max_pages, total_pages, st);
    KvPack pk{nullptr, nullptr};
    if (sealed) {
        TRY(hb.get(&kp, pk_n)); TRY(hb.get(&vp, pk_n));
        launch_kv_seal_all(kc, vc, kp, vp, total_pages, nkv, 1, nullptr, st);
        pk = KvPack{kp, vp};
    }
    const QkvFuse fz{slabs, ksplit, Npad, (const uint16_t*)dev_qnw, (const uint16_t*)dev_knw, (const uint16_t*)dev_cos, (const uint16_t*)dev_sin, eps};
    const float scale = 1.0f / sqrtf((float)MTTS_HD);
    if (path == 1) {
        if (attn_row_prepare()) return fail(MTTS_EINVAL, "attn_row_kernel: the dynamic LDS limit could not be raised");
        if (!attn_row_fits(nq / nkv, &fz, sealed ? &pk : nullptr, pages_bound)) return fail(MTTS_EINVAL, "attn_section: the whole-row kernel does not take this shape");
    }
    if (const int rc = launch_attn(nullptr, kc, vc, pt, meta, scores, stats, opart, outp, MTTS_MAXR, pages_bound, max_pages, total_pages, nch,
                                   nq, nkv, scale, &fz, path == 1 ? ATTN_ROW : ATTN_ALL, st, sealed ? &pk : nullptr))
        return fail(MTTS_EINVAL, rc == -2 ? "attn_section: the whole-row kernel does not take this shape" : "attention group size not built (1, 2, 4)");
    HIPCHK(hipGetLastError());
    HIPCHK(hipMemcpyAsync(dev_out, outp, (size_t)MTTS_MAXR * nq * MTTS_HD * 2, hipMemcpyDeviceToDevice, st));
    HIPCHK(hipMemcpyAsync(dev_kcache, kc, cache_n * 2, hipMemcpyDeviceToDevice, st));
    HIPCHK(hipMemcpyAsync(dev_vcache, vc, cache_n * 2, hipMemcpyDeviceToDevice, st));
    if (sealed && dev_kpack) HIPCHK(hipMemcpyAsync(dev_kpack, kp, pk_n, hipMemcpyDeviceToDevice, st));
    if (sealed && dev_vpack) HIPCHK(hipMemcpyAsync(dev_vpack, vp, pk_n, hipMemcpyDeviceToDevice, st));
    HIPCHK(hipStreamSynchronize(st));
    return MTTS_OK;
}
int64_t mtts_debug_attn_row_launches(void) { return (int64_t)mtts_attn_row_launches(); }

int32_t mtts_k_attn_prefill(const float* dev_slabs, int32_t ksplit, const void* dev_qnw, const void* dev_knw, const void* dev_cos,
                            const void* dev_sin, float eps, const void* dev_k, const void* dev_v, const int32_t* host_lens,
                            const int32_t* host_cached, const int32_t* host_page_table, int32_t B, int32_t Lmax, int32_t nq,
                            int32_t nkv, void* dev_out, void* dev_q, void* dev_kcache, void* dev_vcache, void* stream) {
    if (!dev_slabs || !dev_qnw || !dev_knw || !dev_cos || !dev_sin || !dev_k || !dev_v || !host_lens || !host_cached || !dev_out ||
        !dev_q || !dev_kcache || !dev_vcache || B < 1 || B > MTTS_RCAP || Lmax < 1 || nq < 1 || nkv < 1 || nq % nkv || ksplit < 1 || ksplit > 8)
        return fail(MTTS_EINVAL, "attn_prefill: bad argument (1..%d dialogues, nq %% nkv == 0, 1 <= ksplit <= 8)", MTTS_RCAP);
    if (const int G = nq / nkv; G != 1 && G != 2 && G != 4) return fail(MTTS_EINVAL, "attention group size not built (1, 2, 4)");
    const int max_pages = pages_for(Lmax), total_pages = B * max_pages, nch = (max_pages + ATT_PB - 1) / ATT_PB;
    const int nch_pf = (max_pages + ATT_PF - 1) / ATT_PF, Npad = (nq + 2 * nkv) * MTTS_HD;
    int64_t M = 0;
    int pages_bound = 1;
    for (int b = 0; b < B; ++b) {
        const int n = host_lens[b], c = host_cached[b];
        if (c < 0 || c % MTTS_MAXR || c >= n || n > Lmax)
            return fail(MTTS_EINVAL, "attn_prefill: dialogue %d: need cached %% 32 == 0 and 0 <= cached (%d) < lens (%d) <= Lmax (%d)", b, c, n, Lmax);
        M += round_up(n - c, MTTS_MAXR);
        pages_bound = std::max(pages_bound, pages_for(n));
    }
    if (M > MTTS_PFCAP) return fail(MTTS_EINVAL, "attn_prefill: %lld staged rows, a pass holds %d", (long long)M, MTTS_PFCAP);
    std::vector<int32_t> hpt((size_t)total_pages);
    std::vector<char> seen(total_pages, 0);
    for (size_t i = 0; i < hpt.size(); ++i) {
        hpt[i] = host_page_table ? host_page_table[i] : (int32_t)i;
        if (hpt[i] < 0 || hpt[i] >= total_pages || seen[hpt[i]]) return fail(MTTS_EINVAL, "page table must be a permutation of 0..%d", total_pages - 1);
        seen[hpt[i]] = 1;
    }
    const int R = round_up((int)M, MTTS_RCAP);
    std::vector<RowMeta> hm(R, RowMeta{-1, 0, 0, 0});
    {
        int r = 0;
        for (int b = 0; b < B; r = round_up(r, MTTS_MAXR), ++b)
            for (int i = host_cached[b]; i < host_lens[b]; ++i, ++r) hm[r] = RowMeta{b, i, i == host_lens[b] - 1 ? 1 : 0, 0};
    }
    hipStream_t st = S(stream);
    RowMeta* meta = nullptr; int32_t *pt = nullptr, *lens = nullptr; uint16_t *kc = nullptr, *vc = nullptr, *qbuf = nullptr, *scores = nullptr, *outp = nullptr;
    float *stats = nullptr, *opart = nullptr, *slabs = nullptr;
    const size_t cache_n = (size_t)total_pages * nkv * MTTS_PAGE * MTTS_HD;
    const size_t q_n = (size_t)R * nq * MTTS_HD, sc_n = (size_t)R * nq * max_pages * MTTS_PAGE, st_n = (size_t)R * nq * max_pages * 2;
    const size_t op_n = (size_t)R * nq * nch_pf * MTTS_HD, sl_n = (size_t)ksplit * MTTS_PFCAP * Npad;
    DevBufs hb;
    TRY(hb.get(&meta, (size_t)R, false)); TRY(hb.get(&pt, hpt.size(), false)); TRY(hb.get(&lens, (size_t)B, false));
    TRY(hb.get(&kc, cache_n)); TRY(hb.get(&vc, cache_n));
    TRY(hb.get(&qbuf, q_n, false)); TRY(hb.get(&scores, sc_n, false)); TRY(hb.get(&stats, st_n, false)); TRY(hb.get(&opart, op_n, false));
    TRY(hb.get(&outp, q_n, false)); TRY(hb.get(&slabs, sl_n, false));
    HIPCHK(hipMemsetAsync(qbuf, 0xff, q_n * 2, st)); HIPCHK(hipMemsetAsync(scores, 0xff, sc_n * 2, st));
    HIPCHK(hipMemsetAsync(stats, 0xff, st_n * 4, st)); HIPCHK(hipMemsetAsync(opart, 0xff, op_n * 4, st));
    HIPCHK(hipMemsetAsync(outp, 0xff, q_n * 2, st)); HIPCHK(hipMemsetAsync(slabs, 0xff, sl_n * 4, st));
    std::vector<int32_t> full(B, Lmax);
    HIPCHK(hipMemcpyAsync(meta, hm.data(), hm.size() * sizeof(RowMeta), hipMemcpyHostToDevice, st));
    HIPCHK(hipMemcpyAsync(pt, hpt.data(), hpt.size() * 4, hipMemcpyHostToDevice, st));
    HIPCHK(hipMemcpyAsync(lens, full.data(), (size_t)B * 4, hipMemcpyHostToDevice, st));
    for (int k = 0; k < ksplit; ++k)
        HIPCHK(hipMemcpyAsync(slabs + (size_t)k * MTTS_PFCAP * Npad, dev_slabs + (size_t)k * M * Npad, (size_t)M * Npad * 4, hipMemcpyDeviceToDevice, st));
    launch_pack_kv_pages(dev_k, dev_v, kc, vc, pt, lens, B, Lmax, nkv, max_pages, total_pages, st);
    const float scale = 1.0f / sqrtf((float)MTTS_HD);
    launch_qkv_post(slabs, ksplit, Npad, meta, dev_qnw, dev_knw, dev_cos, dev_sin, qbuf, kc, vc, pt, max_pages, total_pages, R, nq, nkv, eps, st);
    static const AttnPhase prefill_ph[3] = {ATTN_PF_SCORES, ATTN_PF_PV, ATTN_PF_COMBINE};
    for (int i = 0; i < 3; ++i)
        if (launch_attn(qbuf, kc, vc, pt, meta, scores, stats, opart, outp, R, pages_bound, max_pages, total_pages, nch, nq, nkv, scale,
                        nullptr, prefill_ph[i], st, nullptr))
            return fail(MTTS_EINVAL, "attention group size not built (1, 2, 4)");
    launch_unpack_rows(outp, dev_out, (int)M, nq * MTTS_HD, st);
    HIPCHK(hipGetLastError());
    HIPCHK(hipMemcpyAsync(dev_q, qbuf, (size_t)M * nq * MTTS_HD * 2, hipMemcpyDeviceToDevice, st));
    HIPCHK(hipMemcpyAsync(dev_kcache, kc, cache_n * 2, hipMemcpyDeviceToDevice, st));
    HIPCHK(hipMemcpyAsync(dev_vcache, vc, cache_n * 2, hipMemcpyDeviceToDevice, st));
    HIPCHK(hipStreamSynchronize(st));
    return MTTS_OK;
}

int32_t mtts_k_kv_seal(const void* dev_pages, int32_t npages, void* dev_sealed, int32_t as_k, void* stream) {
    if (!dev_pages || !dev_sealed || npages < 1) return fail(MTTS_EINVAL, "kv_seal: bad argument");
    launch_kv_seal_pages(dev_pages, dev_sealed, npages, as_k, S(stream));
    HIPCHK(hipGetLastError());
    HIPCHK(hipStreamSynchronize(S(stream)));
    return MTTS_OK;
}

int32_t mtts_debug_kv_pack_stats(MttsEngine* e, int64_t* out6) {
    if (!e || !out6) return fail(MTTS_EINVAL, "null argument");
    if (!e->kpack) return fail(MTTS_ESTATE, "the engine keeps no sealed pages (fp32 / fp16 engine, or MTTS_KV_PACK=0)");
    HIPCHK(hipSetDevice(e->device));
    HIPCHK(hipDeviceSynchronize());
    std::vector<SeqState> ss(MTTS_RCAP);
    HIPCHK(hipMemcpy(ss.data(), e->d_seqs, ss.size() * sizeof(SeqState), hipMemcpyDeviceToHost));
    std::vector<int32_t> complete(e->B, 0);
    for (int b = 0; b < e->B; ++b)
        if (e->slot_live[b]) complete[b] = std::min(ss[b].kv_len >> 6, e->pool.pages_of(b));
    DevBufs hb;
    int32_t* dc = nullptr; unsigned long long* dout = nullptr;
    TRY(hb.get(&dc, e->B)); TRY(hb.get(&dout, 4));
    HIPCHK(hipMemcpy(dc, complete.data(), e->B * 4, hipMemcpyHostToDevice));
    HIPCHK(hipMemset(dout, 0, 32));
    launch_kv_pack_count(e->kpack, e->vpack, e->d_page_table, dc, e->B, e->max_pages, e->total_pages, e->nkv, e->L, dout, nullptr);
    HIPCHK(hipGetLastError());
    unsigned long long h[4];
    HIPCHK(hipMemcpy(h, dout, 32, hipMemcpyDeviceToHost));
    for (int i = 0; i < 4; ++i) out6[i] = (int64_t)h[i];
    out6[4] = out6[5] = 0;
    for (int n = 0; n < e->L; ++n) { out6[4] += e->pack_k_on[n]; out6[5] += e->pack_v_on[n]; }
    return MTTS_OK;
}

int32_t mtts_debug_set_kv_len(MttsEngine* e, int32_t kv_len) {
    if (!e || !e->began) return fail(MTTS_ESTATE, "mtts_begin has not run");
    if (e->f32) return fail(MTTS_EINVAL, "measurement hook of the bf16 engine");
    HIPCHK(hipSetDevice(e->device));
    HIPCHK(hipDeviceSynchronize());
    const int cap = std::min(e->max_pages * MTTS_PAGE, e->bufs.rope_rows);
    const int limit = cap - MTTS_PAGE;
    if (kv_len < 1 || kv_len > limit) return fail(MTTS_EINVAL, "kv_len %d outside 1..%d", kv_len, limit);
    e->max_steps = std::min(e->max_steps, e->steps_issued + cap - kv_len);
    std::vector<SeqState> ss(MTTS_RCAP);
    HIPCHK(hipMemcpy(ss.data(), e->d_seqs, ss.size() * sizeof(SeqState), hipMemcpyDeviceToHost));
    for (int b = 0; b < e->B; ++b) { ss[b].kv_len = kv_len; e->n_real[b] = kv_len - e->steps_issued; }
    e->max_real = kv_len - e->steps_issued;
    HIPCHK(hipMemcpy(e->d_seqs, ss.data(), ss.size() * sizeof(SeqState), hipMemcpyHostToDevice));
    launch_fill_random_bf16(e->kcache, e->layer_stride * e->L, 0x1234u, nullptr);
    launch_fill_random_bf16(e->vcache, e->layer_stride * e->L, 0x9876u, nullptr);
    if (e->kpack) launch_kv_seal_all(e->kcache, e->vcache, e->kpack, e->vpack, e->total_pages, e->nkv, e->L, nullptr, nullptr);
    HIPCHK(hipDeviceSynchronize());
    return MTTS_OK;
}

int32_t mtts_k_attn_bench(MttsEngine* e, int32_t phase, int32_t iters, float* avg_ms, int64_t* bytes_per_launch) {
    if (!e || !e->began || phase < ATTN_ALL || phase > ATTN_ROW || iters < 1 || !avg_ms) return fail(MTTS_EINVAL, "attn_bench: bad argument");
    if (e->f32) return fail(MTTS_EINVAL, "measurement hook of the bf16 engine");
    HIPCHK(hipSetDevice(e->device));
    HIPCHK(hipDeviceSynchronize());
    const float scale = 1.0f / sqrtf((float)MTTS_HD);
    const int R = round_up(e->B, 32);
    const int len_bound = e->max_real + e->steps_issued + 1;
    const int pages_bound = pages_for(len_bound);
    const StepPlan plan = decode_plan(e, pages_bound);
    if (phase == ATTN_ROW) {
        if (attn_row_prepare()) return fail(MTTS_EINVAL, "attn_row_kernel: the dynamic LDS limit could not be raised");
        const QkvFuse f0{e->bufs.partial, e->p_qkv.ksplit, e->qkv_rows, nullptr, nullptr, nullptr, nullptr, 0.f};
        for (int n = 0; n < e->L; ++n) {
            const KvPack pk = layer_pack(e, plan, n);
            if (!attn_row_fits(e->nq / e->nkv, &f0, (pk.k || pk.v) ? &pk : nullptr, pages_bound))
                return fail(MTTS_EINVAL, "attn_bench: the whole-row kernel does not take this shape");
        }
    }
    hipEvent_t e0, e1;
    hipEventCreate(&e0); hipEventCreate(&e1);
    auto run = [&](int n) {
        for (int i = 0; i < n; ++i) {
            const int layer = i % e->L;
            uint16_t* kc = (uint16_t*)e->kcache + e->layer_stride * layer;
            uint16_t* vc = (uint16_t*)e->vcache + e->layer_stride * layer;
            const QkvFuse fz{e->bufs.partial, e->p_qkv.ksplit, e->qkv_rows, (const uint16_t*)e->layers[layer].qn,
                             (const uint16_t*)e->layers[layer].kn, e->bufs.rope_cos, e->bufs.rope_sin, e->cfg.rms_norm_eps};
            const KvPack pk = layer_pack(e, plan, layer);
            launch_attn(e->qbuf, kc, vc, e->d_page_table, e->d_meta, e->scores, e->stats, e->opart, e->attn_p, R, pages_bound,
                        e->max_pages, e->total_pages, e->nchunks_max, e->nq, e->nkv, scale, (phase == ATTN_ROW || e->B * pages_bound <= e->knobs.fuse_qkv_max) ? &fz : nullptr, (AttnPhase)phase, nullptr,
                        (pk.k || pk.v) ? &pk : nullptr);
        }
    };
    run(e->L);
    hipEventRecord(e0, nullptr);
    run(iters);
    hipEventRecord(e1, nullptr);
    HIPCHK(hipEventSynchronize(e1));
    float ms = 0;
    hipEventElapsedTime(&ms, e0, e1);
    *avg_ms = ms / iters;
    if (bytes_per_launch) {
        std::vector<RowMeta> m(MTTS_RCAP);
        HIPCHK(hipMemcpy(m.data(), e->d_meta, m.size() * sizeof(RowMeta), hipMemcpyDeviceToHost));
        int64_t tok = 0;
        for (int b = 0; b < R; ++b) if (m[b].seq >= 0) tok += m[b].pos + 1;
        *bytes_per_launch = phase == ATTN_COMBINE ? 0 : tok * e->nkv * MTTS_HD * 2 * ((phase == ATTN_ALL || phase == ATTN_ROW) ? 2 : 1);
    }
    hipEventDestroy(e0); hipEventDestroy(e1);
    return MTTS_OK;
}

int32_t mtts_k_gemm_bench(int32_t N, int32_t K, int32_t epi, int32_t ksplit, int32_t waves, int32_t copies,
                                     int32_t iters, float* avg_us) {
    if (N % 32 || K % 16 || copies < 1 || iters < 1 || !avg_us) return fail(MTTS_EINVAL, "gemm_bench: bad argument");
    const int tile_rows = waves < 0 ? -waves : 0;
    if (tile_rows > MTTS_PFCAP) return fail(MTTS_EINVAL, "gemm_bench: at most MTTS_PFCAP rows");
    GemmPlan p = (ksplit > 0 && waves > 0) ? mtts_plan_gemm_forced(N, K, ksplit, waves) : mtts_plan_gemm(N, K, tile_rows ? std::max(ksplit, 1) : ksplit);
    if (tile_rows) p.ksplit = std::max(ksplit, 1);
    p.depth = gemm_depth_env();
    DevBufs hb;
    std::vector<uint16_t*> w(copies, nullptr);
    for (auto& q : w) { TRY(hb.get(&q, (size_t)N * K, false)); HIPCHK(hipMemset(q, 0x3c, (size_t)N * K * 2)); }
    uint16_t *x = nullptr, *out = nullptr;
    float* part = nullptr;
    TRY(hb.get(&x, (size_t)MTTS_PFCAP * K, false));
    HIPCHK(hipMemset(x, 0x3c, (size_t)MTTS_PFCAP * K * 2));
    TRY(hb.get(&out, (size_t)MTTS_PFCAP * N));
    TRY(hb.get(&part, (size_t)p.ksplit * MTTS_PFCAP * N));
    hipEvent_t e0, e1;
    hipEventCreate(&e0); hipEventCreate(&e1);
    auto go = [&](int i) {
        if (tile_rows) launch_gemm_tile(epi, tile_rows, p.ksplit, w[i % copies], x, K, N, N, part, out, nullptr);
        else launch_gemm(epi, 1, p, w[i % copies], x, K, N, N, part, out, nullptr);
    };
    for (int i = 0; i < copies; ++i) go(i);
    HIPCHK(hipDeviceSynchronize());
    hipEventRecord(e0, nullptr);
    for (int i = 0; i < iters; ++i) go(i);
    hipEventRecord(e1, nullptr);
    HIPCHK(hipEventSynchronize(e1));
    float ms = 0;
    hipEventElapsedTime(&ms, e0, e1);
    *avg_us = ms * 1000.f / iters;
    hipEventDestroy(e0); hipEventDestroy(e1);
    return MTTS_OK;
}

int64_t mtts_debug_fold_norm_launches(void) { return (int64_t)mtts_fold_norm_launches(); }

static int fold_hook_args(const char* who, int R, int N) {
    if (R < 1 || R > 32 || N < 32 || N % 32) return fail(MTTS_EINVAL, "%s: need 1<=R<=32, N%%32==0 (K is 2048)", who);
    return MTTS_OK;
}

int32_t mtts_k_oproj_resid(const void* dev_wo, const void* dev_attn, void* dev_x, void* dev_x_packed, int32_t R, int32_t N,
                           void* stream) {
    if (!dev_wo || !dev_attn || !dev_x || !dev_x_packed) return fail(MTTS_EINVAL, "oproj_resid: null argument");
    TRY(fold_hook_args("oproj_resid", R, N));
    hipStream_t st = S(stream);
    const int K = 2048;
    uint16_t *wp = nullptr, *ap = nullptr;
    DevBufs hb;
    TRY(hb.get(&wp, (size_t)N * K));
    TRY(hb.get(&ap, (size_t)32 * K));
    launch_pack_weight(dev_wo, wp, N, K, N, 1, 0, st);
    launch_pack_rows(dev_attn, ap, R, K, 1, st);
    launch_oproj_resid(wp, ap, dev_x, dev_x_packed, R, N, st);
    HIPCHK(hipGetLastError());
    HIPCHK(hipStreamSynchronize(st));
    return MTTS_OK;
}

int32_t mtts_k_fold_pair(const void* dev_wo, const void* dev_attn, void* dev_x, const void* dev_norm_w, const void* dev_wgu,
// ... 226 lines not shown
```

moss-ttsd_amd/csrc/launch.h:

```cpp
#pragma once
#include <type_traits>

#include "../../include/mtts.h"
#include "common.h"
#include "kvpool.h"

enum { EPI_PARTIAL = 0, EPI_BF16 = 1, EPI_SILU = 2,
       EPI_SILU_RM = 3 };
struct GemmPlan {
    int waves, ksplit, kt_per_split, kt_per_wave;
    int depth;
};
GemmPlan mtts_plan_gemm(int Npad, int K, int want_ksplit);
GemmPlan mtts_plan_gemm_forced(int Npad, int K, int ksplit, int waves);
void launch_gemm(int epi, int mb, const GemmPlan& p, const void* Wp, const void* Xp, int K, int Npad, int n_valid,
                 float* partial, uint16_t* out, hipStream_t st);
int mtts_gemm_form(int epi, int mb, const GemmPlan& p, int K, int Npad, int n_valid);
int mtts_tile_ksplit(int Npad, int K, int R);
void launch_gemm_tile(int epi, int R, int ksplit, const void* Wp, const void* Xp, int K, int Npad, int n_valid,
                      float* partial, uint16_t* out, hipStream_t st);
int mtts_small_lds_bytes(const GemmPlan& p, int K, int pro);
void launch_gemv_small(int epi, int pro, const GemmPlan& p, const void* Wp, int K, int Npad, int n_valid, float* partial,
                       uint16_t* out, const SmallPro& pr, hipStream_t st);
long long mtts_gemm_depth_launches();
void mtts_gemm_depth_note();
void launch_pack_weight(const void* src, void* dst, int rows, int cols, int rows_pad, int row_mul, int row_off, hipStream_t st);
void launch_pack_rows(const void* src, void* dst, int R, int K, int tiles, hipStream_t st);
void launch_reduce_partial_bf16(const float* partial, void* out, int ksplit, int Npad, int n_valid, int R, hipStream_t st);

bool wseal_shape(const GemmPlan& p, int K, int Npad, int epi);
size_t wseal_bytes(int Npad, int K, int ktw);
void launch_wseal(const void* Wp, void* Ws, int K, int ktw, int nt0, int ntiles, hipStream_t st);
void launch_wseal_count(const void* Ws, int Npad, int K, int ktw, unsigned long long* out2, hipStream_t st);
bool launch_gemm_sealed(int epi, int mb, const GemmPlan& p, const void* Ws, const void* Wp, const void* Xp, int K, int Npad,
                        int n_valid, float* partial, uint16_t* out, int head_form, hipStream_t st);
long long mtts_wseal_launches();

bool fold_norm_shape(const GemmPlan& p_o, int K_o, const GemmPlan& p_gu, int H, int N_gu);
void launch_oproj_resid(const void* Wp, const void* Xp, void* x, void* x_packed, int R, int N, hipStream_t st);
void launch_gateup_norm(const void* Wp, const void* x_packed, const void* norm_w, float eps, void* out, int Npad, hipStream_t st);
long long mtts_fold_norm_launches();

void launch_embed_norm(const int32_t* tokens, const RowMeta* meta, const uint16_t* const* tables, const void* norm_w,
                       void* x, void* xn_packed, int R, int H, float eps, hipStream_t st);
void launch_resid_norm(const float* partial, int ksplit, int Npad, void* x, const void* norm_w, void* xn_packed,
                       void* hlast, const RowMeta* meta, int R, int H, float eps, hipStream_t st);
void launch_qkv_post(const float* partial, int ksplit, int Npad, const RowMeta* meta, const void* qnw, const void* knw,
                     const void* cosb, const void* sinb, void* qbuf, void* kcache, void* vcache,
                     const int32_t* page_table, int max_pages, int total_pages, int R, int nq, int nkv, float eps,
                     hipStream_t st);
void launch_rmsnorm_rows(const void* x, const void* w, void* y, int rows, int n, float eps, hipStream_t st);
void launch_fill_random_bf16(void* p, size_t n, uint32_t seed, hipStream_t st);
void launch_set_pages(int32_t* table, const PageEdits& ed, hipStream_t st);
void launch_fork(void* kc, void* vc, size_t layer_bytes, size_t head_bytes, int blk_bytes, int L, int nkv, const ForkJob& job,
                 hipStream_t st);
void launch_pack_kv_pages(const void* K, const void* V, void* kcache, void* vcache, const int32_t* page_table, const int32_t* lens,
                          int S, int Lmax, int nkv, int max_pages, int total_pages, hipStream_t st);
void launch_bf16_to_f32(const void* a, float* b, size_t n, hipStream_t st);
void launch_unpack_rows(const void* packed, void* out, int R, int K, hipStream_t st);
void launch_bf16_round_check(unsigned long long* cnt2, hipStream_t st);

enum AttnPhase { ATTN_ALL = 0, ATTN_SCORES = 1, ATTN_PV = 2, ATTN_COMBINE = 3,
                 ATTN_ROW = 4,
                 ATTN_PF_SCORES = 11, ATTN_PF_PV = 12, ATTN_PF_COMBINE = 13 };
int launch_attn(const void* qbuf, void* kcache, void* vcache, const int32_t* page_table,
                const RowMeta* meta, void* scores, float* stats, float* opart, void* out_packed, int R,
                int pages_bound, int max_pages, int total_pages, int nchunks_max, int nq, int nkv, float scale,
                const QkvFuse* fuse, AttnPhase phase, hipStream_t st, const KvPack* pack = nullptr);
bool attn_row_fits(int G, const QkvFuse* fuse, const KvPack* pack, int pages_bound);
int attn_row_prepare();
int attn_row_lds_limit();
long long mtts_attn_row_launches();
void launch_kv_seal_rows(const void* kcache, const void* vcache, void* kpack, void* vpack, const int32_t* page_table,
                         const RowMeta* meta, int R, int max_pages, int total_pages, int nkv, int L, unsigned long long* cnt, hipStream_t st);
void launch_kv_seal_all(const void* kcache, const void* vcache, void* kpack, void* vpack, int total_pages, int nkv, int L,
                        unsigned long long* cnt, hipStream_t st);
void launch_kv_seal_pages(const void* raw, void* pk, int npages, int as_k, hipStream_t st);
void launch_kv_pack_count(const void* kpack, const void* vpack, const int32_t* page_table, const int32_t* complete, int B, int max_pages,
                          int total_pages, int nkv, int L, unsigned long long* out, hipStream_t st);

struct SeqState {
    int32_t nas;
    int32_t unfinished;
    int32_t kv_len;
    int32_t step;
    int32_t base_length;
    int32_t max_length;
    int32_t row_id;
    int32_t active;
    uint64_t seed;
};

struct LoopState {
    int32_t step;
    int32_t done;
    int32_t continuous;
    int32_t B;
    int32_t error;
    int32_t gen_cap;
    int32_t forced_draw;
    int32_t logits_f32;
};
static_assert(sizeof(SeqState) == 40 && std::is_trivially_copyable<SeqState>::value, "SeqState layout");
static_assert(sizeof(LoopState) == 32 && std::is_trivially_copyable<LoopState>::value, "LoopState layout");

#define SAMP_CAND 4096
#define SAMP_NS 32
struct SampleScratch {
    uint32_t* hist = nullptr;
    float* slice_val = nullptr;
    int32_t* slice_idx = nullptr;
    float* cand_val = nullptr;
    int32_t* cand_idx = nullptr;
    uint32_t* cand_n = nullptr;
    int32_t* overflow = nullptr;
    float* full_val = nullptr;
    int32_t* full_idx = nullptr;
    uint32_t* nuc_cnt = nullptr;
    unsigned long long* nuc_mass = nullptr;
    float* slice_sum = nullptr;
    float* lp = nullptr;
    const uint32_t* ban = nullptr;
};
void launch_sample(const void* logits0, const void* logits17, int V0, int Vs, int Vs_pad, const uint32_t* bitmaps,
                   int bm_words, const MttsSamplerCfg* cfgs, const LoopState* ls, const SeqState* seqs, uint64_t seed,
                   int32_t* decisions, int32_t* err, int B, const SampleScratch& sc, int ch0_sampled, int full_cap,
                   int emit_lp, const MttsSamplerFloors* floors ,
                   const float* typical , hipStream_t st);
void launch_sample_single(const void* logits, int rows, int vocab, const uint32_t* bitmap, int bm_words,
                          const MttsSamplerCfg* cfgs8, int mask_id, uint64_t seed, int step, int channel,
                          int32_t* decisions, int32_t* err, const SampleScratch& sc, int full_cap, int emit_lp,
                          const MttsSamplerFloors* floors8, const float* typical8, hipStream_t st);
struct BanCfg { int32_t ngram, eos_below; };
void launch_ban(uint32_t* ban, const uint32_t* stat, int words, const BanCfg* cfgs, const int32_t* hist, int hist_cap,
                const int32_t* gen, int V0, int Vs, int eos, const LoopState* ls, const SeqState* seqs, int B, hipStream_t st);
void launch_ban_single(uint32_t* ban, const uint32_t* stat, const BanCfg* cfg1, const int32_t* hist, const int32_t* lens, int rows,
                       int cap, int vocab, int eos, hipStream_t st);
long long mtts_ban_launches();
struct GenTopkOut {
    int32_t k = 0;
    float* logp = nullptr;
    int32_t* ids = nullptr;
    float* tlp = nullptr;
};
void launch_update(const int32_t* decisions, int32_t* dec_log, const int32_t* forced, const int32_t* tf_tail,
                   int32_t* gen, int32_t* cur_tokens, SeqState* seqs, RowMeta* meta, uint32_t* bitmaps, int bm_words,
                   LoopState* ls, int eos, int spad, int sp_lo, int sp_hi, const float* lp_in, float* lp_out,
                   const GenTopkOut& gt, hipStream_t st);
void launch_export_codes(const int32_t* gen, int64_t* codes, int B, int first, int n, int speech_offset, int clamp_hi,
                         int cap, hipStream_t st);

// ... 60 lines not shown
```

moss-ttsd_amd/mtts/capi.py:

```python
from __future__ import annotations

import ctypes as C
import os

_HERE = os.path.dirname(os.path.abspath(__file__))
LIB_PATH = os.path.join(os.path.dirname(_HERE), "lib", "libmtts.so")


class MttsConfig(C.Structure):
    _fields_ = [(n, C.c_int32) for n in (
        "vocab_size", "hidden_size", "intermediate_size", "num_hidden_layers", "num_attention_heads",
        "num_key_value_heads", "head_dim", "channels", "speech_vocab_size", "speech_pad_token",
        "speech_range_lo", "speech_range_hi", "eos_token_id", "max_position")] + [
        ("rms_norm_eps", C.c_float), ("max_batch", C.c_int32), ("max_seq_len", C.c_int32), ("kv_pool_pages", C.c_int32), ("dtype", C.c_int32)]


class MttsSamplerCfg(C.Structure):
    _fields_ = [("do_sample", C.c_int32), ("top_k", C.c_int32), ("top_p", C.c_float),
                ("one_minus_top_p", C.c_float), ("temperature", C.c_float), ("repetition_penalty", C.c_float)]


class MttsSamplerFloors(C.Structure):
    _fields_ = [("min_p", C.c_float), ("epsilon_cutoff", C.c_float), ("eta_cutoff", C.c_float), ("sqrt_eta_cutoff", C.c_float)]

# ... 32 lines not shown
    "mtts_engine_create": (C.c_int32, [C.POINTER(MttsConfig), C.c_int32, C.POINTER(C.c_void_p)]),
    "mtts_engine_destroy": (C.c_int32, [C.c_void_p]),
    "mtts_bind_weight": (C.c_int32, [C.c_void_p, C.c_char_p, C.c_void_p, C.c_int64, C.c_int64, C.c_void_p]),
    "mtts_bind_weight_lora": (C.c_int32, [C.c_void_p, C.c_char_p, C.c_void_p, C.c_int64, C.c_int64, C.c_void_p, C.c_void_p,
                                          C.c_int32, C.c_float, C.c_void_p]),
    "mtts_k_lora_pack": (C.c_int32, [C.c_void_p, C.c_int32, C.c_int32, C.c_void_p, C.c_void_p, C.c_int32, C.c_float,
                                     C.c_int32, C.c_int32, C.c_int32, C.c_int32, C.c_void_p, C.c_void_p]),
    "mtts_adapter_load": (C.c_int32, [C.c_void_p, C.c_int32, C.c_char_p, C.c_void_p, C.c_void_p, C.c_int64, C.c_int64, C.c_int32,
                                      C.c_float, C.c_void_p]),
    "mtts_adapter_clear": (C.c_int32, [C.c_void_p, C.c_int32]),
    "mtts_set_row_adapters": (C.c_int32, [C.c_void_p, C.c_void_p, C.c_int32]),
    "mtts_set_slot_adapter": (C.c_int32, [C.c_void_p, C.c_int32, C.c_int32]),
    "mtts_k_lora_delta": (C.c_int32, [C.c_void_p, C.c_int32, C.c_int32, C.c_int32, C.c_int32, C.c_void_p, C.c_int32] +
                          [C.c_void_p] * 6 + [C.c_int32, C.c_void_p]),
    "mtts_k_swiglu_slabs": (C.c_int32, [C.c_void_p] * 5 + [C.c_int32] * 3 + [C.c_void_p]),
    "mtts_bind_rope": (C.c_int32, [C.c_void_p, C.c_void_p, C.c_void_p, C.c_int32, C.c_void_p]),
    "mtts_weights_ready": (C.c_int32, [C.c_void_p]),
    "mtts_generate": (C.c_int32, [C.c_void_p, C.c_void_p, C.c_void_p, C.c_int32, C.c_int32, C.c_int32,
                                  C.POINTER(MttsSamplerCfg), C.c_uint64, C.c_void_p, C.c_int32,
                                  C.POINTER(C.c_int32), C.c_void_p, C.c_int32, C.c_void_p, C.c_void_p]),
    "mtts_begin": (C.c_int32, [C.c_void_p, C.c_void_p, C.c_void_p, C.c_int32, C.c_int32, C.c_int32,
                               C.POINTER(MttsSamplerCfg), C.c_uint64, C.c_void_p]),
    "mtts_step": (C.c_int32, [C.c_void_p, C.c_int32, C.c_void_p]),
    "mtts_sync_state": (C.c_int32, [C.c_void_p, C.POINTER(C.c_int32), C.POINTER(C.c_int32), C.c_void_p]),
    "mtts_read_generated": (C.c_int32, [C.c_void_p, C.c_void_p, C.c_int32, C.POINTER(C.c_int32)]),
    "mtts_set_output_scores": (C.c_int32, [C.c_void_p, C.c_int32]),
    "mtts_read_scores": (C.c_int32, [C.c_void_p, C.c_void_p, C.c_int32, C.POINTER(C.c_int32)]),
    "mtts_slot_read_scores": (C.c_int32, [C.c_void_p, C.c_int32, C.c_void_p, C.c_int32, C.POINTER(C.c_int32)]),
    "mtts_set_top_logprobs": (C.c_int32, [C.c_void_p, C.c_int32]),
    "mtts_read_top_logprobs": (C.c_int32, [C.c_void_p, C.c_void_p, C.c_void_p, C.c_void_p, C.c_int32, C.POINTER(C.c_int32)]),
    "mtts_slot_read_top_logprobs": (C.c_int32, [C.c_void_p, C.c_int32, C.c_void_p, C.c_void_p, C.c_void_p, C.c_int32,
                                                C.POINTER(C.c_int32)]),
    "mtts_k_gen_topk": (C.c_int32, [C.c_void_p, C.c_int32, C.c_int32, C.c_int32, C.c_int32, C.c_void_p, C.c_int32, C.c_void_p,
                                    C.c_void_p, C.c_void_p, C.c_void_p]),
    "mtts_score": (C.c_int32, [C.c_void_p, C.c_void_p, C.c_void_p, C.c_void_p, C.c_int32, C.c_int32, C.c_void_p, C.c_void_p]),
    "mtts_score_topk": (C.c_int32, [C.c_void_p, C.c_void_p, C.c_void_p, C.c_void_p, C.c_int32, C.c_int32, C.c_void_p, C.c_int32,
                                    C.c_void_p, C.c_void_p, C.c_void_p]),
    "mtts_read_logits": (C.c_int32, [C.c_void_p, C.c_void_p, C.c_void_p, C.c_void_p]),
    "mtts_read_logits_f32": (C.c_int32, [C.c_void_p, C.c_void_p, C.c_void_p, C.c_void_p]),
    "mtts_sched_open": (C.c_int32, [C.c_void_p, C.c_int32, C.c_int32, C.POINTER(MttsSamplerCfg), C.c_void_p]),
    "mtts_slot_submit": (C.c_int32, [C.c_void_p, C.c_int32, C.c_void_p, C.c_int32, C.c_int32, C.c_uint64, C.c_void_p]),
    "mtts_slot_submit_row": (C.c_int32, [C.c_void_p, C.c_int32, C.c_void_p, C.c_int32, C.c_int32, C.c_uint64, C.c_int32, C.c_void_p]),
    "mtts_set_row_ids": (C.c_int32, [C.c_void_p, C.c_void_p, C.c_int32]),
    "mtts_set_takes": (C.c_int32, [C.c_void_p, C.c_int32]),
    "mtts_set_sampler_floors": (C.c_int32, [C.c_void_p, C.POINTER(MttsSamplerFloors)]),
    "mtts_set_sampler_bans": (C.c_int32, [C.c_void_p, C.POINTER(MttsSamplerBans)]),
    "mtts_set_sampler_typical": (C.c_int32, [C.c_void_p, C.POINTER(C.c_float)]),
    "mtts_debug_ban_launches": (C.c_int64, []),
    "mtts_slot_fork": (C.c_int32, [C.c_void_p, C.c_int32, C.c_int32, C.c_uint64, C.c_int32, C.c_void_p]),
    "mtts_slot_states": (C.c_int32, [C.c_void_p, C.c_void_p, C.c_void_p]),
    "mtts_slot_read": (C.c_int32, [C.c_void_p, C.c_int32, C.c_void_p, C.c_int32, C.POINTER(C.c_int32)]),
    "mtts_read_seq_state": (C.c_int32, [C.c_void_p, C.c_void_p, C.c_void_p, C.c_void_p, C.c_void_p]),
    "mtts_slot_evict": (C.c_int32, [C.c_void_p, C.c_int32, C.c_void_p]),
    "mtts_kv_pool_state": (C.c_int32, [C.c_void_p, C.POINTER(C.c_int32), C.POINTER(C.c_int32), C.POINTER(C.c_int32)]),
    "mtts_read_page_table": (C.c_int32, [C.c_void_p, C.c_void_p, C.c_void_p]),
    "mtts_set_forced_mode": (C.c_int32, [C.c_void_p, C.c_int32]),
    "mtts_debug_read_device_page_table": (C.c_int32, [C.c_void_p, C.c_void_p, C.c_void_p]),
    "mtts_export_codes": (C.c_int32, [C.c_void_p, C.c_int32, C.c_int32, C.c_void_p, C.c_void_p]),
    "mtts_profile_enable": (C.c_int32, [C.c_void_p, C.c_int32]),
    "mtts_profile_read": (C.c_int32, [C.c_void_p, C.c_int32, C.POINTER(C.c_double), C.POINTER(C.c_int64),
                                      C.POINTER(C.c_int64)]),
    "mtts_debug_set_kv_len": (C.c_int32, [C.c_void_p, C.c_int32]),
    "mtts_debug_kv_pack_stats": (C.c_int32, [C.c_void_p, C.c_void_p]),
    "mtts_debug_step_plan": (C.c_int32, [C.c_void_p, C.c_int32, C.c_char_p, C.c_int32]),
    "mtts_k_kv_seal": (C.c_int32, [C.c_void_p, C.c_int32, C.c_void_p, C.c_int32, C.c_void_p]),
    "mtts_k_attn_bench": (C.c_int32, [C.c_void_p, C.c_int32, C.c_int32, C.POINTER(C.c_float), C.POINTER(C.c_int64)]),
    "mtts_k_gemm_bench": (C.c_int32, [C.c_int32] * 7 + [C.POINTER(C.c_float)]),
    "mtts_k_gemm_bf16": (C.c_int32, [C.c_void_p, C.c_void_p, C.c_void_p, C.c_int32, C.c_int32, C.c_int32,
                                     C.c_int32, C.c_void_p]),
    "mtts_debug_gemm_depth_launches": (C.c_int64, []),
    "mtts_debug_wseal_launches": (C.c_int64, []),
    "mtts_debug_wseal_stats": (C.c_int32, [C.c_void_p, C.c_void_p]),
    "mtts_k_wseal": (C.c_int32, [C.c_void_p, C.c_int32, C.c_int32, C.c_int32, C.c_void_p, C.c_void_p]),
    "mtts_k_gemm_sealed": (C.c_int32, [C.c_void_p, C.c_void_p, C.c_void_p] + [C.c_int32] * 7 + [C.c_void_p, C.c_void_p]),
    "mtts_k_gemm_sealed_bench": (C.c_int32, [C.c_void_p] + [C.c_int32] * 8 + [C.POINTER(C.c_float), C.c_void_p]),
    "mtts_debug_attn_row_launches": (C.c_int64, []),
    "mtts_debug_fold_norm_launches": (C.c_int64, []),
    "mtts_k_oproj_resid": (C.c_int32, [C.c_void_p] * 4 + [C.c_int32] * 2 + [C.c_void_p]),
    "mtts_k_fold_pair": (C.c_int32, [C.c_void_p] * 5 + [C.c_float] + [C.c_int32] * 2 + [C.c_void_p, C.c_void_p]),
    "mtts_k_bf16_round_check": (C.c_int32, [C.c_void_p, C.c_void_p]),
    "mtts_k_fold_bench": (C.c_int32, [C.c_int32] * 4 + [C.POINTER(C.c_float)]),
    "mtts_k_attn_section": (C.c_int32, [C.c_void_p, C.c_int32] + [C.c_void_p] * 4 + [C.c_float] + [C.c_void_p] * 4 +
                            [C.c_int32] * 6 + [C.c_void_p] * 6),
    "mtts_k_attn_prefill": (C.c_int32, [C.c_void_p, C.c_int32] + [C.c_void_p] * 4 + [C.c_float] + [C.c_void_p] * 5 +
                            [C.c_int32] * 4 + [C.c_void_p] * 5),
    "mtts_k_gemm_swiglu_bf16": (C.c_int32, [C.c_void_p, C.c_void_p, C.c_void_p, C.c_int32, C.c_int32, C.c_int32, C.c_void_p]),
    "mtts_k_rmsnorm": (C.c_int32, [C.c_void_p, C.c_void_p, C.c_void_p, C.c_int32, C.c_int32, C.c_float, C.c_void_p]),
    "mtts_k_embed_norm": (C.c_int32, [C.c_void_p] * 5 + [C.c_int32, C.c_int32, C.c_float] + [C.c_void_p] * 3),
    "mtts_k_resid_norm": (C.c_int32, [C.c_void_p, C.c_int32, C.c_int32] + [C.c_void_p] * 4 + [C.c_int32] * 3 + [C.c_float] +
                          [C.c_void_p] * 3),
    "mtts_k_gemv_small": (C.c_int32, [C.c_int32, C.c_int32, C.c_void_p] + [C.c_int32] * 4 + [C.c_void_p, C.c_void_p, C.c_int32,
                                      C.c_void_p, C.c_float] + [C.c_void_p] * 4 + [C.c_int32, C.c_int32] + [C.c_void_p] * 4),
    "mtts_k_gemm_tile": (C.c_int32, [C.c_int32] + [C.c_void_p] * 3 + [C.c_int32] * 4 + [C.c_void_p]),
    "mtts_k_rope_kvwrite": (C.c_int32, [C.c_void_p] * 6 + [C.c_int32, C.c_int32, C.c_int32, C.c_float] + [C.c_void_p] * 4),
    "mtts_k_paged_attn_decode": (C.c_int32, [C.c_void_p] * 5 + [C.c_int32] * 4 + [C.c_void_p, C.c_void_p]),
    "mtts_k_head_ce": (C.c_int32, [C.c_void_p, C.c_void_p, C.c_void_p] + [C.c_int32] * 5 + [C.c_void_p, C.c_void_p]),
    "mtts_k_head_topk": (C.c_int32, [C.c_void_p, C.c_void_p] + [C.c_int32] * 6 + [C.c_void_p, C.c_void_p, C.c_void_p]),
    "mtts_k_sample": (C.c_int32, [C.c_void_p, C.c_int32, C.c_int32, C.c_void_p, C.POINTER(MttsSamplerCfg),
                                  C.c_int32, C.c_uint64, C.c_int32, C.c_int32, C.c_void_p, C.c_void_p]),
    "mtts_k_sample_scores": (C.c_int32, [C.c_void_p, C.c_int32, C.c_int32, C.c_void_p, C.POINTER(MttsSamplerCfg),
                                         C.c_int32, C.c_uint64, C.c_int32, C.c_int32, C.c_void_p, C.c_void_p, C.c_void_p]),
    "mtts_k_sample_floors": (C.c_int32, [C.c_void_p, C.c_int32, C.c_int32, C.c_void_p, C.POINTER(MttsSamplerCfg),
                                         C.c_int32, C.c_uint64, C.c_int32, C.c_int32, C.c_void_p, C.c_void_p,
                                         C.POINTER(MttsSamplerFloors), C.c_void_p]),
    "mtts_k_sample_bans": (C.c_int32, [C.c_void_p, C.c_int32, C.c_int32, C.c_void_p, C.POINTER(MttsSamplerCfg),
                                       C.c_int32, C.c_uint64, C.c_int32, C.c_int32, C.c_void_p, C.c_void_p,
                                       C.POINTER(MttsSamplerFloors), C.c_void_p, C.c_void_p]),
    "mtts_k_sample_typical": (C.c_int32, [C.c_void_p, C.c_int32, C.c_int32, C.c_void_p, C.POINTER(MttsSamplerCfg),
                                          C.c_int32, C.c_uint64, C.c_int32, C.c_int32, C.c_void_p, C.c_void_p,
                                          C.POINTER(MttsSamplerFloors), C.c_void_p, C.c_float, C.c_void_p]),
    "mtts_k_ngram_ban": (C.c_int32, [C.c_void_p, C.c_void_p, C.c_int32, C.c_int32, C.c_int32, C.c_void_p, C.c_int32, C.c_int32,
                                     C.c_int32, C.c_int32, C.c_void_p, C.c_void_p]),
    "mtts_codec_last_error": (C.c_char_p, []),
    "mtts_codec_create": (C.c_int32, [C.POINTER(MttsCodecConfig), C.c_int32, C.POINTER(C.c_void_p)]),
    "mtts_codec_destroy": (C.c_int32, [C.c_void_p]),
    "mtts_codec_bind": (C.c_int32, [C.c_void_p, C.c_char_p, C.c_void_p, C.c_int64, C.c_void_p]),
    "mtts_codec_detokenize": (C.c_int32, [C.c_void_p, C.c_void_p, C.c_void_p, C.c_int32, C.c_int32, C.c_void_p, C.c_void_p]),
    "mtts_codec_detokenize_async": (C.c_int32, [C.c_void_p, C.c_void_p, C.c_void_p, C.c_int32, C.c_int32, C.c_void_p, C.c_void_p]),
    "mtts_codec_check": (C.c_int32, [C.c_void_p, C.c_void_p]),
    "mtts_codec_tokenize": (C.c_int32, [C.c_void_p, C.c_void_p, C.c_void_p, C.c_int32, C.c_int32, C.c_void_p, C.c_void_p, C.c_void_p]),
    "mtts_k_gemm_f32": (C.c_int32, [C.c_void_p, C.c_void_p, C.c_void_p, C.c_void_p, C.c_int32, C.c_int32, C.c_int32,
                                    C.c_int32, C.c_void_p]),
    "mtts_k_gemm_planes_bench": (C.c_int32, [C.c_int32, C.c_int32, C.c_int32, C.c_int32, C.c_int32, C.c_int32,
                                             C.POINTER(C.c_float), C.POINTER(C.c_int32)]),
    "mtts_k_codec_attn": (C.c_int32, [C.c_void_p] * 3 + [C.c_int32] * 5 + [C.c_void_p]),
    "mtts_k_codec_gemm_planes": (C.c_int32, [C.c_void_p] * 6 + [C.c_int32] * 9 + [C.c_void_p]),
    "mtts_k_codec_vocos_pw": (C.c_int32, [C.c_void_p] * 7 + [C.c_int32, C.c_void_p]),
    "mtts_k_codec_layernorm": (C.c_int32, [C.c_void_p] * 4 + [C.c_int32, C.c_int32, C.c_float, C.c_void_p] + [C.c_int32] * 3 +
                               [C.c_void_p]),
    "mtts_k_codec_layernorm_wide": (C.c_int32, [C.c_void_p] * 4 + [C.c_int32, C.c_int32, C.c_float, C.c_void_p]),
    "mtts_k_codec_dwconv_ln": (C.c_int32, [C.c_void_p] * 6 + [C.c_int32] * 3 + [C.c_float, C.c_int32, C.c_int32, C.c_void_p]),
    "mtts_k_codec_softmax_mask": (C.c_int32, [C.c_void_p, C.c_void_p] + [C.c_int32] * 4 + [C.c_void_p]),
    "mtts_k_codec_vq_argmin_update": (C.c_int32, [C.c_void_p] * 6 + [C.c_int32] * 4 + [C.c_void_p]),
    "mtts_k_codec_gemm_f32_ex": (C.c_int32, [C.c_void_p] * 6 + [C.c_int32] * 4 + [C.c_int64] * 4 + [C.c_int32, C.c_int32, C.c_float,
                                                                                                   C.c_int32, C.c_int32, C.c_void_p,
                                                                                                   C.c_void_p]),
}


def exported_symbols():
    return sorted(_SIGS)


def lib():
    global _lib
    if _lib is None:
        if not os.path.exists(LIB_PATH):
            raise MttsError(f"{LIB_PATH} is missing: build it with `python moss-ttsd_amd/build.py` "
                            "(hipcc --offload-arch=gfx950); there is no CPU fallback")
        L = C.CDLL(LIB_PATH)
        for name, (res, args) in _SIGS.items():
            fn = getattr(L, name)
            fn.restype = res
            fn.argtypes = args
        _lib = L
    return _lib


def check(rc):
    if rc != 0:
        raise MttsError(f"libmtts error {rc}: {lib().mtts_last_error().decode()}", rc)
```

Measured before the change: 83660 codec_tokens/s.

## Prefetch page IDs into registers and overlap epilogue loads with first KV request

The whole-row attention kernel now loads the sequence's page-table entries into per-lane registers before the metadata check, using a speculative row index. It fetches page IDs with readlane instead of global loads per page. The fused QKV epilogue is split so that norm weights, partial sums and rope values are requested early and the first K page load is issued before the epilogue math, hiding latency behind the stage barrier. bf16 rounding is also done in pairs via a packed round helper, and a slot-permutation test entry point is added. The cost is more register pressure from the register-held page table, plus a redundant reload when the speculation misses.

```diff
diff --git a/include/mtts.h b/include/mtts.h
--- a/include/mtts.h
+++ b/include/mtts.h
@@ -172,6 +172,11 @@
                             const int32_t* host_page_table, int32_t R, int32_t Lmax, int32_t nq, int32_t nkv, int32_t sealed,
                             int32_t path, void* dev_out, void* dev_kcache, void* dev_vcache, void* dev_kpack, void* dev_vpack,
                             void* stream);
+int32_t mtts_k_attn_section_slots(const float* dev_slabs, int32_t ksplit, const void* dev_qnw, const void* dev_knw, const void* dev_cos,
+                                  const void* dev_sin, float eps, const void* dev_k, const void* dev_v, const int32_t* host_lens,
+                                  const int32_t* host_page_table, const int32_t* host_slots, int32_t R, int32_t Lmax, int32_t nq,
+                                  int32_t nkv, int32_t sealed, int32_t path, void* dev_out, void* dev_kcache, void* dev_vcache,
+                                  void* dev_kpack, void* dev_vpack, void* stream);
 int32_t mtts_k_attn_prefill(const float* dev_slabs, int32_t ksplit, const void* dev_qnw, const void* dev_knw, const void* dev_cos,
                             const void* dev_sin, float eps, const void* dev_k, const void* dev_v, const int32_t* host_lens,
                             const int32_t* host_cached, const int32_t* host_page_table, int32_t B, int32_t Lmax, int32_t nq,
diff --git a/moss-ttsd_amd/csrc/attn.hip b/moss-ttsd_amd/csrc/attn.hip
--- a/moss-ttsd_amd/csrc/attn.hip
+++ b/moss-ttsd_amd/csrc/attn.hip
@@ -2,6 +2,7 @@
 #include <algorithm>
 #include <atomic>
 #include <cstdlib>
+#include <type_traits>
 #ifndef MTTS_PK_WAVES
 #define MTTS_PK_WAVES 0
 #endif
@@ -12,6 +13,7 @@
 #endif
 
 #include "seal.h"
+#include "norm_ops.h"
 
 __device__ bool seal_lane_k(const u32x4_t* __restrict__ raw, u32x4_t* __restrict__ pk, uint8_t* __restrict__ lds, int lane) {
     u32x4_t v[16];
@@ -244,8 +246,9 @@
         for (int j = 0; j < 8; ++j)
             if (k0 + j < f.ksplit && k0 + j > 0) { a += ta[j]; b += tb[j]; }
     }
-    a = rbf(a);
-    b = rbf(b);
+    const uint32_t t = pack2_rn(a, b);
+    a = bflo(t);
+    b = bfhi(t);
 }
 
 __device__ __forceinline__ void fuse_reduce_request(const QkvFuse& f, int r, int col, int lane, float (&ta)[8], float (&tb)[8]) {
@@ -263,8 +266,9 @@
 #pragma unroll
     for (int j = 1; j < 8; ++j)
         if (j < f.ksplit) { a += ta[j]; b += tb[j]; }
-    a = rbf(a);
-    b = rbf(b);
+    const uint32_t t = pack2_rn(a, b);
+    a = bflo(t);
+    b = bfhi(t);
 }
 
 struct FuseVec { float w0, w1, c, s; };
@@ -279,10 +283,25 @@
 __device__ __forceinline__ void fuse_norm_rope(const QkvFuse& f, const FuseVec& v, float a, float b, float& o1, float& o2) {
     const float ss = wave_sum(a * a + b * b);
     const float inv = 1.0f / sqrtf(ss / (float)MTTS_HD + f.eps);
-    a = rbf(v.w0 * rbf(a * inv));
-    b = rbf(v.w1 * rbf(b * inv));
-    o1 = rbf(rbf(a * v.c) + rbf(-b * v.s));
-    o2 = rbf(rbf(b * v.c) + rbf(a * v.s));
+    const uint32_t n = pack2_rn(a * inv, b * inv);
+    const uint32_t w = pack2_rn(v.w0 * bflo(n), v.w1 * bfhi(n));
+    a = bflo(w);
+    b = bfhi(w);
+    const uint32_t p1 = pack2_rn(a * v.c, -b * v.s), p2 = pack2_rn(b * v.c, a * v.s);
+    const uint32_t o = pack2_rn(bflo(p1) + bfhi(p1), bflo(p2) + bfhi(p2));
+    o1 = bflo(o);
+    o2 = bfhi(o);
+}
+__device__ __forceinline__ uint16_t bf_bits(float rounded) { return (uint16_t)(__float_as_uint(rounded) >> 16); }
+template <int G>
+__device__ __forceinline__ void score_round(const float* acc, float scale, float (&s)[G]) {
+#pragma unroll
+    for (int g = 0; g < G; g += 2) {
+        const uint32_t t = pack2_rn(acc[g], g + 1 < G ? acc[g + 1] : 0.f);
+        const uint32_t u = pack2_rn(bflo(t) * scale, bfhi(t) * scale);
+        s[g] = bflo(u);
+        if (g + 1 < G) s[g + 1] = bfhi(u);
+    }
 }
 
 template <int G, bool FUSED, bool PK>
@@ -338,16 +357,16 @@
                 }
                 fuse_norm_rope(f, fv, a, b, o1, o2);
                 if (!isk) {
-                    ((uint16_t*)qs[hh])[lane] = f2bf(o1);
-                    ((uint16_t*)qs[hh])[lane + 64] = f2bf(o2);
+                    ((uint16_t*)qs[hh])[lane] = bf_bits(o1);
+                    ((uint16_t*)qs[hh])[lane + 64] = bf_bits(o2);
                 } else {
-                    knew[lane] = f2bf(o1);
-                    knew[lane + 64] = f2bf(o2);
+                    knew[lane] = bf_bits(o1);
+                    knew[lane + 64] = bf_bits(o2);
                     const int opage = page_table[(size_t)m.seq * max_pages + own_pg];
                     uint16_t* base = (uint16_t*)kcache + ((size_t)kvh * total_pages + opage) * (MTTS_PAGE * MTTS_HD);
                     const int tok = m.pos & 63;
-                    base[(((lane >> 3) * 64) + tok) * 8 + (lane & 7)] = f2bf(o1);
-                    base[((((lane + 64) >> 3) * 64) + tok) * 8 + (lane & 7)] = f2bf(o2);
+                    base[(((lane >> 3) * 64) + tok) * 8 + (lane & 7)] = bf_bits(o1);
+                    base[((((lane + 64) >> 3) * 64) + tok) * 8 + (lane & 7)] = bf_bits(o2);
                 }
             }
         } else {
@@ -362,11 +381,13 @@
     auto finish = [&](const float* acc) {
         const int tok = pg * MTTS_PAGE + lane;
         const bool valid = tok < len;
+        float sr[G];
+        score_round<G>(acc, scale, sr);
 #pragma unroll
         for (int g = 0; g < G; ++g) {
             const int h = kvh * G + g;
-            float sc = rbf(rbf(acc[g]) * scale);
-            if (valid) scores[((size_t)r * nq + h) * Lmax + tok] = f2bf(sc);
+            const float sc = sr[g];
+            if (valid) scores[((size_t)r * nq + h) * Lmax + tok] = bf_bits(sc);
             float mx = wave_max(valid ? sc : -INFINITY);
             float e = valid ? expf(sc - mx) : 0.f;
             float sm = wave_sum(e);
@@ -525,13 +546,13 @@
         float a, b;
         if (pre_v) fuse_reduce_sum(f, vta, vtb, a, b);
         else fuse_reduce(f, r, (nq + nkv + kvh) * MTTS_HD, lane, a, b);
-        vnew[lane] = f2bf(a);
-        vnew[lane + 64] = f2bf(b);
+        vnew[lane] = bf_bits(a);
+        vnew[lane + 64] = bf_bits(b);
         const int page = page_table[(size_t)m.seq * max_pages + own_pg];
         const int tok = m.pos & 63;
         uint16_t* dst = (uint16_t*)vcache + ((size_t)kvh * total_pages + page) * (MTTS_PAGE * MTTS_HD) + (size_t)(tok >> 1) * (MTTS_HD * 2) + (tok & 1);
-        dst[2 * lane] = f2bf(a);
-        dst[2 * (lane + 64)] = f2bf(b);
+        dst[2 * lane] = bf_bits(a);
+        dst[2 * (lane + 64)] = bf_bits(b);
     }
     float M[G], S[G];
 #pragma unroll
@@ -676,12 +697,14 @@
 static std::atomic<long long> g_row_launches{0};
 long long mtts_attn_row_launches() { return g_row_launches.load(); }
 
+constexpr int row_pid_regs(int G) { return G == 1 ? 7 : G == 2 ? 4 : 2; }
+
 template <int G, bool PK>
 __global__ __launch_bounds__(ROW_WAVES * 64) void attn_row_kernel(
     u32x4_t* __restrict__ kcache, u32x4_t* __restrict__ vcache, const int32_t* __restrict__ page_table,
     const RowMeta* __restrict__ meta, uint16_t* __restrict__ out_packed, int npb, int max_pages, int total_pages, int nq,
-    int nkv, float scale, QkvFuse f, const u32x4_t* __restrict__ kpack, const u32x4_t* __restrict__ vpack) {
-    constexpr int W = ROW_WAVES;
+    int nkv, float scale, QkvFuse f, const u32x4_t* __restrict__ kpack, const u32x4_t* __restrict__ vpack, int table_rows) {
+    constexpr int W = ROW_WAVES, NPID = row_pid_regs(G);
     extern __shared__ __attribute__((aligned(16))) uint8_t row_lds[];
     uint32_t* qs = (uint32_t*)row_lds;
     uint16_t* knew = (uint16_t*)(row_lds + G * 256);
@@ -692,63 +715,101 @@
     uint16_t* sc = (uint16_t*)(st + G * npb);
     float* items = (float*)(sc + (size_t)G * npb * MTTS_PAGE);
     const int r = blockIdx.y, kvh = blockIdx.x;
+    const int wave = __builtin_amdgcn_readfirstlane(threadIdx.x >> 6), lane = threadIdx.x & 63;
+    const int sub = lane >> 5, dl = lane & 31;
+    const bool epi = wave < G + 2;
+    const int vw = epi ? wave + W - (G + 2) : wave - (G + 2);
+    const int col = (wave < G ? kvh * G + wave : wave == G ? nq + kvh : nq + nkv + kvh) * MTTS_HD;
+
     const RowMeta m = meta[r];
+    const int srow = r < table_rows ? r : 0;
+    typedef int32_t pid_t __attribute__((ext_vector_type(NPID)));
+    pid_t pid;
+    auto load_ids = [&](int row) {
+        const int32_t* t = page_table + (size_t)row * max_pages;
+#pragma unroll
+        for (int j = 0; j < NPID; ++j) pid[j] = t[min(lane + 64 * j, npb - 1)];
+    };
+    load_ids(srow);
+    int32_t first_id = page_table[(size_t)srow * max_pages + min(vw, npb - 1)];
+    uint16_t nw0 = 0, nw1 = 0, rc = 0, rs = 0;
+    float pta[8], ptb[8];
+    if (epi) {
+        const uint16_t* nw = wave == G ? f.knorm_w : f.qnorm_w;
+        nw0 = nw[lane];
+        nw1 = nw[lane + 64];
+        if (f.ksplit <= 8) fuse_reduce_request(f, r, col, lane, pta, ptb);
+    }
+    __builtin_amdgcn_sched_barrier(0);
+    asm volatile("" : "+s"(first_id));
     if (m.seq < 0) {
         for (int i = threadIdx.x; i < G * MTTS_HD; i += W * 64) out_packed[xpack_off(r, kvh * G * MTTS_HD + i, nq * MTTS_HD)] = f2bf(0.f);
         return;
     }
+    if (m.seq != srow) {
+        load_ids(m.seq);
+        first_id = page_table[(size_t)m.seq * max_pages + min(vw, npb - 1)];
+    }
     const int len = m.pos + 1;
     const int npages = min((len + MTTS_PAGE - 1) / MTTS_PAGE, npb);
     const int nch = (npages + ATT_PB - 1) / ATT_PB;
-    const int wave = __builtin_amdgcn_readfirstlane(threadIdx.x >> 6), lane = threadIdx.x & 63;
     const int own_pg = m.pos >> 6;
-    const int sub = lane >> 5, dl = lane & 31;
-    const int32_t* ptab = page_table + (size_t)m.seq * max_pages;
-
-    const bool epi = wave < G + 2;
-    const int vw = epi ? wave + W - (G + 2) : wave - (G + 2);
-    if (epi) {
-        const int col = (wave < G ? kvh * G + wave : wave == G ? nq + kvh : nq + nkv + kvh) * MTTS_HD;
-        FuseVec pfv{0.f, 0.f, 0.f, 0.f};
-        if (wave <= G) pfv = fuse_load_vec(f, wave == G ? f.knorm_w : f.qnorm_w, m.pos, lane);
+    auto pid_at = [&](int pg) {
+        int32_t v = pid[0];
+#pragma unroll
+        for (int j = 1; j < NPID; ++j) v = (pg >> 6) == j ? pid[j] : v;
+        return __builtin_amdgcn_readlane(v, pg & 63);
+    };
+
+    auto rope_request = [&]() {
+        rc = f.rope_cos[(size_t)m.pos * 64 + lane];
+        rs = f.rope_sin[(size_t)m.pos * 64 + lane];
+    };
+    auto epilogue = [&]() {
         float a, b;
-        if (f.ksplit <= 8) {
-            float pta[8], ptb[8];
-            fuse_reduce_request(f, r, col, lane, pta, ptb);
-            fuse_reduce_sum(f, pta, ptb, a, b);
-        } else fuse_reduce(f, r, col, lane, a, b);
-        const int opage = ptab[own_pg], tok = m.pos & 63;
+        if (f.ksplit <= 8) fuse_reduce_sum(f, pta, ptb, a, b);
+        else fuse_reduce(f, r, col, lane, a, b);
+        const int opage = pid_at(own_pg), tok = m.pos & 63;
         if (wave <= G) {
             float o1, o2;
-            fuse_norm_rope(f, pfv, a, b, o1, o2);
+            fuse_norm_rope(f, FuseVec{bf2f(nw0), bf2f(nw1), bf2f(rc), bf2f(rs)}, a, b, o1, o2);
             if (wave < G) {
-                ((uint16_t*)(qs + wave * 64))[lane] = f2bf(o1);
-                ((uint16_t*)(qs + wave * 64))[lane + 64] = f2bf(o2);
+                ((uint16_t*)(qs + wave * 64))[lane] = bf_bits(o1);
+                ((uint16_t*)(qs + wave * 64))[lane + 64] = bf_bits(o2);
             } else {
-                knew[lane] = f2bf(o1);
-                knew[lane + 64] = f2bf(o2);
+                knew[lane] = bf_bits(o1);
+                knew[lane + 64] = bf_bits(o2);
                 uint16_t* base = (uint16_t*)kcache + ((size_t)kvh * total_pages + opage) * (MTTS_PAGE * MTTS_HD);
-                base[(((lane >> 3) * 64) + tok) * 8 + (lane & 7)] = f2bf(o1);
-                base[((((lane + 64) >> 3) * 64) + tok) * 8 + (lane & 7)] = f2bf(o2);
+                base[(((lane >> 3) * 64) + tok) * 8 + (lane & 7)] = bf_bits(o1);
+                base[((((lane + 64) >> 3) * 64) + tok) * 8 + (lane & 7)] = bf_bits(o2);
             }
         } else {
-            vnew[lane] = f2bf(a);
-            vnew[lane + 64] = f2bf(b);
+            asm volatile("" ::"v"(rc), "v"(rs));
+            vnew[lane] = bf_bits(a);
+            vnew[lane + 64] = bf_bits(b);
             uint16_t* dst = (uint16_t*)vcache + ((size_t)kvh * total_pages + opage) * (MTTS_PAGE * MTTS_HD) + (size_t)(tok >> 1) * (MTTS_HD * 2) + (tok & 1);
-            dst[2 * lane] = f2bf(a);
-            dst[2 * (lane + 64)] = f2bf(b);
-        }
-        __builtin_amdgcn_sched_barrier(0);
-    }
-    auto stage = [&]() { __syncthreads(); };
+            dst[2 * lane] = bf_bits(a);
+            dst[2 * (lane + 64)] = bf_bits(b);
+        }
+    };
+    auto stage = [&](auto&& request) __attribute__((always_inline)) {
+        if (epi) {
+            rope_request();
+            request();
+            epilogue();
+        } else request();
+        __syncthreads();
+    };
 
     auto finish = [&](int pg, const float* acc) {
         const int tok = pg * MTTS_PAGE + lane;
         const bool valid = tok < len;
+        float sr[G];
+        score_round<G>(acc, scale, sr);
 #pragma unroll
         for (int g = 0; g < G; ++g) {
-            float s = rbf(rbf(acc[g]) * scale);
-            if (valid) sc[(size_t)g * npb * MTTS_PAGE + tok] = f2bf(s);
+            const float s = sr[g];
+            if (valid) sc[(size_t)g * npb * MTTS_PAGE + tok] = bf_bits(s);
             float mx = wave_max(valid ? s : -INFINITY);
             float e = valid ? expf(s - mx) : 0.f;
             float sm = wave_sum(e);
@@ -779,15 +840,19 @@
         }
         finish(pg, acc);
     };
-    auto k_page = [&](int pg, bool first) {
-        const int page = ptab[pg];
+    auto k_page = [&](int pg, auto first_c) __attribute__((always_inline)) {
+        constexpr bool first = decltype(first_c)::value;
+        const int page = first ? first_id : pid_at(pg);
         const u32x4_t* kp = kcache + ((size_t)kvh * total_pages + page) * (MTTS_PAGE * MTTS_HD / 8) + lane;
         if (PK && pg < own_pg) {
             u32x4_t pk[MTTS_PKU];
             const u32x4_t* pp = kpack + ((size_t)kvh * total_pages + page) * (MTTS_PKU * 64) + lane;
-#pragma unroll
-            for (int j = 0; j < MTTS_PKU; ++j) pk[pk_order(j)] = __builtin_nontemporal_load(pp + pk_order(j) * 64);
-            if (first) stage();
+            auto request = [&]() __attribute__((always_inline)) {
+#pragma unroll
+                for (int j = 0; j < MTTS_PKU; ++j) pk[pk_order(j)] = __builtin_nontemporal_load(pp + pk_order(j) * 64);
+            };
+            if (first) stage(request);
+            else request();
             bool qok = true;
             const uint32_t sh = pk[12].z;
             uint32_t* qwv = qw + wave * G * 64;
@@ -839,22 +904,25 @@
             finish(pg, acc);
         } else {
             u32x4_t kv[16];
-#pragma unroll
-            for (int j = 0; j < 16; ++j) kv[j] = __builtin_nontemporal_load(kp + j * 64);
-            if (first) stage();
+            auto request = [&]() __attribute__((always_inline)) {
+#pragma unroll
+                for (int j = 0; j < 16; ++j) kv[j] = __builtin_nontemporal_load(kp + j * 64);
+            };
+            if (first) stage(request);
+            else request();
             raw_dots(pg, kv);
         }
     };
-    if (vw < npages) k_page(vw, true);
-    else stage();
+    if (vw < npages) k_page(vw, std::true_type{});
+    else stage([]() {});
 #pragma unroll 1
-    for (int pg = vw + W; pg < npages; pg += W) k_page(pg, false);
+    for (int pg = vw + W; pg < npages; pg += W) k_page(pg, std::false_type{});
 
     u32x4_t vv[16];
     bool packed = false;
     const u32x4_t* vp = nullptr;
     auto load_page = [&](int pg) {
-        const int page = ptab[pg];
+        const int page = pid_at(pg);
         vp = vcache + ((size_t)kvh * total_pages + page) * (MTTS_PAGE * MTTS_HD / 8) + lane;
         packed = PK && pg < own_pg;
         if (packed) {
@@ -1191,7 +1259,7 @@
 static void launch_attn_g(const void* qbuf, void* kcache, void* vcache, const int32_t* page_table,
                           const RowMeta* meta, void* scores, float* stats, float* opart, void* out_packed, int R,
                           int pages_bound, int max_pages, int total_pages, int nchunks_max, int nq, int nkv, float scale,
-                          const QkvFuse* fuse, AttnPhase phase, hipStream_t st, const KvPack* pack) {
+                          const QkvFuse* fuse, AttnPhase phase, hipStream_t st, const KvPack* pack, int table_rows) {
     if (phase == ATTN_PF_SCORES) {
         dim3 ga((pages_bound + 3) / 4, nkv, R / MTTS_MAXR);
         hipLaunchKernelGGL((attn_prefill_scores_kernel<G>), ga, dim3(256), 0, st, (const uint16_t*)qbuf, (const u32x4_t*)kcache,
@@ -1217,10 +1285,10 @@
         const size_t lds = (size_t)attn_row_lds_bytes(G, kpk != nullptr, pages_bound);
         if (kpk)
             hipLaunchKernelGGL((attn_row_kernel<G, true>), dim3(nkv, R), dim3(ROW_WAVES * 64), lds, st, (u32x4_t*)kcache, (u32x4_t*)vcache,
-                               page_table, meta, (uint16_t*)out_packed, pages_bound, max_pages, total_pages, nq, nkv, scale, f, kpk, vpk);
+                               page_table, meta, (uint16_t*)out_packed, pages_bound, max_pages, total_pages, nq, nkv, scale, f, kpk, vpk, table_rows);
         else
             hipLaunchKernelGGL((attn_row_kernel<G, false>), dim3(nkv, R), dim3(ROW_WAVES * 64), lds, st, (u32x4_t*)kcache, (u32x4_t*)vcache,
-                               page_table, meta, (uint16_t*)out_packed, pages_bound, max_pages, total_pages, nq, nkv, scale, f, kpk, vpk);
+                               page_table, meta, (uint16_t*)out_packed, pages_bound, max_pages, total_pages, nq, nkv, scale, f, kpk, vpk, table_rows);
         g_row_launches.fetch_add(1);
         return;
     }
@@ -1257,6 +1325,7 @@
 bool attn_row_fits(int G, const QkvFuse* fuse, const KvPack* pack, int pages_bound) {
     const bool pk = pack && pack->k;
     if (!fuse || (G != 1 && G != 2 && G != 4) || pk != (pack && pack->v)) return false;
+    if (pages_bound < 1 || pages_bound > 64 * row_pid_regs(G)) return false;
     return attn_row_lds_bytes(G, pk, pages_bound) <= g_row_lds_max;
 }
 int attn_row_prepare() {
@@ -1285,13 +1354,13 @@
 int launch_attn(const void* qbuf, void* kcache, void* vcache, const int32_t* page_table,
                 const RowMeta* meta, void* scores, float* stats, float* opart, void* out_packed, int R,
                 int pages_bound, int max_pages, int total_pages, int nchunks_max, int nq, int nkv, float scale,
-                const QkvFuse* fuse, AttnPhase phase, hipStream_t st, const KvPack* pack) {
+                const QkvFuse* fuse, AttnPhase phase, hipStream_t st, const KvPack* pack, int table_rows) {
     int G = nq / nkv;
     if (G != 1 && G != 2 && G != 4) return -1;
     if (phase == ATTN_ROW && !attn_row_fits(G, fuse, pack, pages_bound)) return -2;
 #define MTTS_ATT(GG)                                                                                              \
     launch_attn_g<GG>(qbuf, kcache, vcache, page_table, meta, scores, stats, opart, out_packed, R, pages_bound,   \
-                      max_pages, total_pages, nchunks_max, nq, nkv, scale, fuse, phase, st, pack)
+                      max_pages, total_pages, nchunks_max, nq, nkv, scale, fuse, phase, st, pack, table_rows)
     if (G == 1) MTTS_ATT(1);
     else if (G == 2) MTTS_ATT(2);
     else if (G == 4) MTTS_ATT(4);
diff --git a/moss-ttsd_amd/csrc/engine.hip b/moss-ttsd_amd/csrc/engine.hip
--- a/moss-ttsd_amd/csrc/engine.hip
+++ b/moss-ttsd_amd/csrc/engine.hip
@@ -611,7 +611,7 @@
         hipEvent_t ev = nullptr;
         prof_begin(e, PROF_SCORES, st, &ev);
         if (const int rc = launch_attn(e->qbuf, kc, vc, e->d_page_table, d_meta, e->scores, e->stats, e->opart, e->attn_p, R, pages_bound,
-                                       e->max_pages, e->total_pages, e->nchunks_max, e->nq, e->nkv, scale, &fz, ATTN_ROW, st, pkp))
+                                       e->max_pages, e->total_pages, e->nchunks_max, e->nq, e->nkv, scale, &fz, ATTN_ROW, st, pkp, e->cfg.max_batch))
             return fail(MTTS_EINVAL, rc == -2 ? "the whole-row attention kernel does not take this launch" : "attention group size not built");
         prof_end(e, st, ev);
         if (e->prof) e->prof_bytes[PROF_SCORES] += 2 * kv_tokens_hint * e->nkv * MTTS_HD * 2;
diff --git a/moss-ttsd_amd/csrc/hooks.hip b/moss-ttsd_amd/csrc/hooks.hip
--- a/moss-ttsd_amd/csrc/hooks.hip
+++ b/moss-ttsd_amd/csrc/hooks.hip
@@ -604,11 +604,11 @@
     return MTTS_OK;
 }
 
-int32_t mtts_k_attn_section(const float* dev_slabs, int32_t ksplit, const void* dev_qnw, const void* dev_knw, const void* dev_cos,
+static int32_t attn_section(const float* dev_slabs, int32_t ksplit, const void* dev_qnw, const void* dev_knw, const void* dev_cos,
                             const void* dev_sin, float eps, const void* dev_k, const void* dev_v, const int32_t* host_lens,
-                            const int32_t* host_page_table, int32_t R, int32_t Lmax, int32_t nq, int32_t nkv, int32_t sealed,
-                            int32_t path, void* dev_out, void* dev_kcache, void* dev_vcache, void* dev_kpack, void* dev_vpack,
-                            void* stream) {
+                            const int32_t* host_page_table, const int32_t* host_slots, int32_t R, int32_t Lmax, int32_t nq, int32_t nkv,
+                            int32_t sealed, int32_t path, void* dev_out, void* dev_kcache, void* dev_vcache, void* dev_kpack,
+                            void* dev_vpack, void* stream) {
     if (!dev_slabs || !dev_qnw || !dev_knw || !dev_cos || !dev_sin || !dev_k || !dev_v || !host_lens || !dev_out || !dev_kcache ||
         !dev_vcache || R < 1 || R > MTTS_MAXR || Lmax < 1 || nq < 1 || nkv < 1 || nq % nkv || ksplit < 1 || (path != 0 && path != 1))
         return fail(MTTS_EINVAL, "attn_section: bad argument (1..32 rows, path 0 or 1)");
@@ -622,23 +622,33 @@
         if (hpt[i] < 0 || hpt[i] >= total_pages || seen[hpt[i]]) return fail(MTTS_EINVAL, "page table must be a permutation of 0..%d", total_pages - 1);
         seen[hpt[i]] = 1;
     }
+    std::vector<int32_t> hps(hpt);
+    if (host_slots) {
+        std::vector<char> used(R, 0);
+        for (int r = 0; r < R; ++r) {
+            const int s = host_slots[r];
+            if (s < 0 || s >= R || used[s]) return fail(MTTS_EINVAL, "attn_section: slots must be a permutation of 0..%d", R - 1);
+            used[s] = 1;
+            std::copy(hpt.begin() + (size_t)r * max_pages, hpt.begin() + (size_t)(r + 1) * max_pages, hps.begin() + (size_t)s * max_pages);
+        }
+    }
     std::vector<RowMeta> hm(MTTS_MAXR, RowMeta{-1, 0, 0, 0});
     std::vector<int32_t> cached(R, 0);
     int pages_bound = 1;
     for (int r = 0; r < R; ++r) {
         if (host_lens[r] < 0 || host_lens[r] > Lmax) return fail(MTTS_EINVAL, "row %d: length %d outside 0..%d", r, host_lens[r], Lmax);
         if (!host_lens[r]) continue;
-        hm[r] = RowMeta{r, host_lens[r] - 1, 1, 0};
+        hm[r] = RowMeta{host_slots ? host_slots[r] : r, host_lens[r] - 1, 1, 0};
         cached[r] = host_lens[r] - 1;
         pages_bound = std::max(pages_bound, pages_for(host_lens[r]));
     }
     pages_bound = std::min(round_up(pages_bound, ATT_PB), max_pages);
-    RowMeta* meta = nullptr; int32_t *pt = nullptr, *lens = nullptr; uint16_t *kc = nullptr, *vc = nullptr, *scores = nullptr, *outp = nullptr;
+    RowMeta* meta = nullptr; int32_t *pt = nullptr, *pts = nullptr, *lens = nullptr; uint16_t *kc = nullptr, *vc = nullptr, *scores = nullptr, *outp = nullptr;
     float *stats = nullptr, *opart = nullptr, *slabs = nullptr;
     uint8_t *kp = nullptr, *vp = nullptr;
     const size_t cache_n = (size_t)total_pages * nkv * MTTS_PAGE * MTTS_HD, pk_n = (size_t)total_pages * nkv * MTTS_PKU * 64 * 16;
     DevBufs hb;
-    TRY(hb.get(&meta, MTTS_MAXR)); TRY(hb.get(&pt, hpt.size())); TRY(hb.get(&lens, R));
+    TRY(hb.get(&meta, MTTS_MAXR)); TRY(hb.get(&pt, hpt.size())); TRY(hb.get(&pts, hps.size())); TRY(hb.get(&lens, R));
     TRY(hb.get(&kc, cache_n)); TRY(hb.get(&vc, cache_n));
     TRY(hb.get(&scores, (size_t)MTTS_MAXR * nq * max_pages * MTTS_PAGE));
     TRY(hb.get(&stats, (size_t)MTTS_MAXR * nq * max_pages * 2));
@@ -647,6 +657,7 @@
     TRY(hb.get(&slabs, (size_t)ksplit * MTTS_PFCAP * Npad, false));
     HIPCHK(hipMemcpyAsync(meta, hm.data(), hm.size() * sizeof(RowMeta), hipMemcpyHostToDevice, st));
     HIPCHK(hipMemcpyAsync(pt, hpt.data(), hpt.size() * 4, hipMemcpyHostToDevice, st));
+    HIPCHK(hipMemcpyAsync(pts, hps.data(), hps.size() * 4, hipMemcpyHostToDevice, st));
     HIPCHK(hipMemcpyAsync(lens, cached.data(), R * 4, hipMemcpyHostToDevice, st));
     for (int k = 0; k < ksplit; ++k)
         HIPCHK(hipMemcpyAsync(slabs + (size_t)k * MTTS_PFCAP * Npad, dev_slabs + (size_t)k * R * Npad, (size_t)R * Npad * 4, hipMemcpyDeviceToDevice, st));
@@ -663,8 +674,8 @@
         if (attn_row_prepare()) return fail(MTTS_EINVAL, "attn_row_kernel: the dynamic LDS limit could not be raised");
         if (!attn_row_fits(nq / nkv, &fz, sealed ? &pk : nullptr, pages_bound)) return fail(MTTS_EINVAL, "attn_section: the whole-row kernel does not take this shape");
     }
-    if (const int rc = launch_attn(nullptr, kc, vc, pt, meta, scores, stats, opart, outp, MTTS_MAXR, pages_bound, max_pages, total_pages, nch,
-                                   nq, nkv, scale, &fz, path == 1 ? ATTN_ROW : ATTN_ALL, st, sealed ? &pk : nullptr))
+    if (const int rc = launch_attn(nullptr, kc, vc, pts, meta, scores, stats, opart, outp, MTTS_MAXR, pages_bound, max_pages, total_pages, nch,
+                                   nq, nkv, scale, &fz, path == 1 ? ATTN_ROW : ATTN_ALL, st, sealed ? &pk : nullptr, R))
         return fail(MTTS_EINVAL, rc == -2 ? "attn_section: the whole-row kernel does not take this shape" : "attention group size not built (1, 2, 4)");
     HIPCHK(hipGetLastError());
     HIPCHK(hipMemcpyAsync(dev_out, outp, (size_t)MTTS_MAXR * nq * MTTS_HD * 2, hipMemcpyDeviceToDevice, st));
@@ -674,6 +685,23 @@
     if (sealed && dev_vpack) HIPCHK(hipMemcpyAsync(dev_vpack, vp, pk_n, hipMemcpyDeviceToDevice, st));
     HIPCHK(hipStreamSynchronize(st));
     return MTTS_OK;
+}
+int32_t mtts_k_attn_section(const float* dev_slabs, int32_t ksplit, const void* dev_qnw, const void* dev_knw, const void* dev_cos,
+                            const void* dev_sin, float eps, const void* dev_k, const void* dev_v, const int32_t* host_lens,
+                            const int32_t* host_page_table, int32_t R, int32_t Lmax, int32_t nq, int32_t nkv, int32_t sealed,
+                            int32_t path, void* dev_out, void* dev_kcache, void* dev_vcache, void* dev_kpack, void* dev_vpack,
+                            void* stream) {
+    return attn_section(dev_slabs, ksplit, dev_qnw, dev_knw, dev_cos, dev_sin, eps, dev_k, dev_v, host_lens, host_page_table, nullptr, R,
+                        Lmax, nq, nkv, sealed, path, dev_out, dev_kcache, dev_vcache, dev_kpack, dev_vpack, stream);
+}
+int32_t mtts_k_attn_section_slots(const float* dev_slabs, int32_t ksplit, const void* dev_qnw, const void* dev_knw, const void* dev_cos,
+                                  const void* dev_sin, float eps, const void* dev_k, const void* dev_v, const int32_t* host_lens,
+                                  const int32_t* host_page_table, const int32_t* host_slots, int32_t R, int32_t Lmax, int32_t nq,
+                                  int32_t nkv, int32_t sealed, int32_t path, void* dev_out, void* dev_kcache, void* dev_vcache,
+                                  void* dev_kpack, void* dev_vpack, void* stream) {
+    if (!host_slots) return fail(MTTS_EINVAL, "attn_section_slots: host_slots is null");
+    return attn_section(dev_slabs, ksplit, dev_qnw, dev_knw, dev_cos, dev_sin, eps, dev_k, dev_v, host_lens, host_page_table, host_slots, R,
+                        Lmax, nq, nkv, sealed, path, dev_out, dev_kcache, dev_vcache, dev_kpack, dev_vpack, stream);
 }
 int64_t mtts_debug_attn_row_launches(void) { return (int64_t)mtts_attn_row_launches(); }
 
@@ -833,7 +861,7 @@
             const KvPack pk = layer_pack(e, plan, layer);
             launch_attn(e->qbuf, kc, vc, e->d_page_table, e->d_meta, e->scores, e->stats, e->opart, e->attn_p, R, pages_bound,
                         e->max_pages, e->total_pages, e->nchunks_max, e->nq, e->nkv, scale, (phase == ATTN_ROW || e->B * pages_bound <= e->knobs.fuse_qkv_max) ? &fz : nullptr, (AttnPhase)phase, nullptr,
-                        (pk.k || pk.v) ? &pk : nullptr);
+                        (pk.k || pk.v) ? &pk : nullptr, e->cfg.max_batch);
         }
     };
     run(e->L);
diff --git a/moss-ttsd_amd/csrc/launch.h b/moss-ttsd_amd/csrc/launch.h
--- a/moss-ttsd_amd/csrc/launch.h
+++ b/moss-ttsd_amd/csrc/launch.h
@@ -66,7 +66,7 @@
 int launch_attn(const void* qbuf, void* kcache, void* vcache, const int32_t* page_table,
                 const RowMeta* meta, void* scores, float* stats, float* opart, void* out_packed, int R,
                 int pages_bound, int max_pages, int total_pages, int nchunks_max, int nq, int nkv, float scale,
-                const QkvFuse* fuse, AttnPhase phase, hipStream_t st, const KvPack* pack = nullptr);
+                const QkvFuse* fuse, AttnPhase phase, hipStream_t st, const KvPack* pack = nullptr, int table_rows = 0);
 bool attn_row_fits(int G, const QkvFuse* fuse, const KvPack* pack, int pages_bound);
 int attn_row_prepare();
 int attn_row_lds_limit();
diff --git a/moss-ttsd_amd/mtts/capi.py b/moss-ttsd_amd/mtts/capi.py
--- a/moss-ttsd_amd/mtts/capi.py
+++ b/moss-ttsd_amd/mtts/capi.py
@@ -138,6 +138,8 @@
     "mtts_k_fold_bench": (C.c_int32, [C.c_int32] * 4 + [C.POINTER(C.c_float)]),
     "mtts_k_attn_section": (C.c_int32, [C.c_void_p, C.c_int32] + [C.c_void_p] * 4 + [C.c_float] + [C.c_void_p] * 4 +
                             [C.c_int32] * 6 + [C.c_void_p] * 6),
+    "mtts_k_attn_section_slots": (C.c_int32, [C.c_void_p, C.c_int32] + [C.c_void_p] * 4 + [C.c_float] + [C.c_void_p] * 5 +
+                                  [C.c_int32] * 6 + [C.c_void_p] * 6),
     "mtts_k_attn_prefill": (C.c_int32, [C.c_void_p, C.c_int32] + [C.c_void_p] * 4 + [C.c_float] + [C.c_void_p] * 5 +
                             [C.c_int32] * 4 + [C.c_void_p] * 5),
     "mtts_k_gemm_swiglu_bf16": (C.c_int32, [C.c_void_p, C.c_void_p, C.c_void_p, C.c_int32, C.c_int32, C.c_int32, C.c_void_p]),
```

New measurement: 84030 codec_tokens/s, median of 6. About the same (+0.4%).
